# xingyizhou/CenterNet

Measured on AMD Instinct MI355X. Metric: images/sec whole-node, 512x512 ctdet, higher is better.
Workload: dtype f32s; 1 GPU; ctdet resdcn_18 512x512, batch 32 per GPU (BASELINE configs[1]), network + fused sigmoid/peak-NMS/top-K decode, K=100; global_batch=32, parallelism=image-sharded x1

## Files before the change

centernet_amd/csrc/cn_conv.hip:

```cpp
#include "cn_internal.h"
#include "cn_tuning.h"
#include <type_traits>

#ifndef CN_IGEMM_F32S_SETS
#define CN_IGEMM_F32S_SETS 1
#endif

namespace {

constexpr int NT = 256;
constexpr int BK = 32;
constexpr int LDT = BK + 4;

enum { A_DENSE = 0, A_STEM = 1, A_DCN = 2, A_DCN_PAD = 3 };
constexpr int STEM_KMAX = 512;

struct IgemmArgs {
    const void *x;
    const void *w;
    const float *bias;
    const float *scale;
    const float *shift;
    const void *residual;
    void *y;
// ... 850 lines not shown
extern "C" size_t cn_packed_conv_weight_elems(int Cout, int Cin, int KH, int KW, int dtype)
{
    const size_t n = packed_elems(Cout, Cin, KH, KW, dtype == CN_DTYPE_F16 ? 64 : 32);
    return (dtype == CN_DTYPE_F32S && ((KH == 3 && KW == 3) || (KH == 1 && KW == 1)) && Cin != 3) ? 2 * n : n;
}

template <typename T>
static int pack_conv_weight_t(const float *w_oihw, void *w_packed, int Cout, int Cin, int KH,
                              int KW, int bke, hipStream_t st)
{
    const int taps = KH * KW;
    const int cout_pad = round_up(Cout, 32);
    if (Cin == 3) {
        const int kpad = round_up(taps * 3, bke);
        const size_t total = (size_t)cout_pad * kpad;
        hipLaunchKernelGGL(pack_stem_weight_kernel<T>, dim3((unsigned)cn_cdiv((int)total, 256)),
                           dim3(256), 0, st, w_oihw, (T *)w_packed, Cout, taps, cout_pad, kpad);
    } else {
        const int cin_pad = round_up(Cin, bke);
        const size_t total = (size_t)taps * cout_pad * cin_pad;
        int blocks = (int)((total + 255) / 256);
        if (blocks > 4096) blocks = 4096;
        hipLaunchKernelGGL(pack_weight_kernel<T>, dim3(blocks), dim3(256), 0, st, w_oihw,
                           (T *)w_packed, Cout, Cin, taps, cout_pad, cin_pad);
    }
    CN_CHECK_LAUNCH();
    return CN_OK;
}

extern "C" int cn_pack_conv_weight(const float *w_oihw, void *w_packed, int Cout, int Cin, int KH,
                                   int KW, int dtype, void *stream)
{
    if (!w_oihw || !w_packed) return CN_ERR_NULL;
    if (Cout <= 0 || Cin <= 0 || KH <= 0 || KW <= 0) return CN_ERR_SHAPE;
    if (dtype == CN_DTYPE_F16)
        return pack_conv_weight_t<_Float16>(w_oihw, w_packed, Cout, Cin, KH, KW, 64, (hipStream_t)stream);
    if (dtype == CN_DTYPE_F32S && Cin != 3) {
        const int taps = KH * KW, cout_pad = round_up(Cout, 32), cin_pad = round_up(Cin, 32);
        const size_t total = (size_t)taps * cout_pad * cin_pad;
        int blocks = (int)((total + 255) / 256);
        if (blocks > 4096) blocks = 4096;
        hipLaunchKernelGGL(pack_weight_f32s_kernel, dim3(blocks), dim3(256), 0, (hipStream_t)stream,
                           w_oihw, (_Float16 *)w_packed, Cout, Cin, taps, cout_pad, cin_pad);
        CN_CHECK_LAUNCH();
        if ((KH == 3 && KW == 3) || (KH == 1 && KW == 1)) {
            hipLaunchKernelGGL(pack_weight_f32s_frag_kernel, dim3(blocks), dim3(256), 0,
                               (hipStream_t)stream, w_oihw, (_Float16 *)w_packed + 2 * total, Cout, Cin,
                               taps, cout_pad / 32, cin_pad / 32);
            CN_CHECK_LAUNCH();
        }
        return CN_OK;
    }
    if (dtype != CN_DTYPE_F32 && dtype != CN_DTYPE_F32S) return CN_ERR_UNSUPPORTED;
    return pack_conv_weight_t<float>(w_oihw, w_packed, Cout, Cin, KH, KW, 32, (hipStream_t)stream);
}

extern "C" int cn_pack_conv_weight_f32(const float *w_oihw, float *w_packed, int Cout, int Cin,
                                       int KH, int KW, void *stream)
{
    return cn_pack_conv_weight(w_oihw, w_packed, Cout, Cin, KH, KW, CN_DTYPE_F32, stream);
}

static int conv_fill_args(const cn_conv_desc *d, IgemmArgs *a)
{
    if (d->B <= 0 || d->H <= 0 || d->W <= 0 || d->Cin <= 0 || d->Cout <= 0 || d->KH <= 0 ||
        d->KW <= 0 || d->stride <= 0 || d->dil <= 0 || d->Ho <= 0 || d->Wo <= 0)
        return CN_ERR_SHAPE;
    const int ho = (d->H + 2 * d->pad_h - (d->dil * (d->KH - 1) + 1)) / d->stride + 1;
    const int wo = (d->W + 2 * d->pad_w - (d->dil * (d->KW - 1) + 1)) / d->stride + 1;
    if (d->oy_mul == 1 && d->ox_mul == 1 && (ho != d->Ho || wo != d->Wo)) return CN_ERR_SHAPE;
    if ((long)d->B * d->H * d->W * (long)(d->in_layout == CN_LAYOUT_NHWC ? d->in_pitch : d->Cin) >=
        (1L << 31))
        return CN_ERR_UNSUPPORTED;
    if ((long)d->B * d->OH * d->OW * (long)(d->out_layout == CN_LAYOUT_NHWC ? d->out_pitch : d->Cout) >=
        (1L << 31))
        return CN_ERR_UNSUPPORTED;
    a->B = d->B; a->H = d->H; a->W = d->W; a->Cin = d->Cin;
    a->Ho = d->Ho; a->Wo = d->Wo; a->Cout = d->Cout;
    a->KH = d->KH; a->KW = d->KW; a->stride = d->stride;
    a->pad_h = d->pad_h; a->pad_w = d->pad_w; a->dil = d->dil;
    a->in_pitch = d->in_pitch; a->out_pitch = d->out_pitch;
    a->OH = d->OH; a->OW = d->OW;
    a->oy_mul = d->oy_mul; a->oy_add = d->oy_add; a->ox_mul = d->ox_mul; a->ox_add = d->ox_add;
    a->relu = d->relu;
    a->M = d->B * d->Ho * d->Wo;
    a->cout_pad = round_up(d->Cout, 32);
    const int f16 = (d->dtype == CN_DTYPE_F16);
    const int f32s = (d->dtype == CN_DTYPE_F32S);
    if (d->dtype != CN_DTYPE_F32 && !f16 && !f32s) return CN_ERR_UNSUPPORTED;
    if (f32s && d->in_layout == CN_LAYOUT_NHWC && !(d->flags & CN_CONV_X_PLAIN) && (d->in_pitch & 31))
        return CN_ERR_UNSUPPORTED;
    if (f32s && d->out_layout == CN_LAYOUT_NHWC && !(d->flags & CN_CONV_Y_PLAIN) && (d->out_pitch & 31))
        return CN_ERR_UNSUPPORTED;
    const int bke = f16 ? 64 : 32, epv = f16 ? 8 : 4;
    if (is_stem(d->Cin, d->in_layout)) {
        a->cin_pad = round_up(d->KH * d->KW * 3, bke);
        if (a->cin_pad > STEM_KMAX) return CN_ERR_UNSUPPORTED;
        a->nchunk = a->cin_pad / bke;
        a->KT = a->nchunk;
    } else {
        if (d->in_layout != CN_LAYOUT_NHWC) return CN_ERR_UNSUPPORTED;
        if ((d->Cin % epv) || (d->in_pitch % epv) || d->in_pitch < d->Cin) return CN_ERR_UNSUPPORTED;
        a->cin_pad = round_up(d->Cin, bke);
        a->nchunk = a->cin_pad / bke;
        a->KT = d->KH * d->KW * a->nchunk;
    }
    return CN_OK;
}

static void dense_tile_class(const cn_conv_desc *d, const IgemmArgs &a, int *cls, bool *bm64)
{
    const int waste128 = cn_cdiv(d->Cout, 128) * 128 - d->Cout;
    const int waste64 = cn_cdiv(d->Cout, 64) * 64 - d->Cout;
    const bool narrow = !cn_knobs.narrow && (waste128 - waste64 >= 64);
    *cls = (d->Cout > 64 && !narrow) ? 2 : (d->Cout > 32 ? 1 : 0);
    const long wgs128 = (long)cn_cdiv(a.M, 128) * cn_cdiv(d->Cout, 128) * (a.zparity ? 4 : 1);
    *bm64 = (*cls == 2) && (cn_knobs.bm ? (cn_knobs.bm == 64) : (wgs128 < 1024 && wgs128 != 512));
}

static int dense_ksplit(const cn_conv_desc *d, const IgemmArgs &a)
{
    if (cn_knobs.nosplit || d->out_layout != CN_LAYOUT_NHWC || is_stem(d->Cin, d->in_layout) ||
        a.zparity)
        return 1;
    int cls;
    bool bm64;
    dense_tile_class(d, a, &cls, &bm64);
    const int bm = bm64 ? 64 : 128, bn = cls == 2 ? 128 : (cls == 1 ? 64 : 32);
    return plan_ksplit(a.M, d->Cout, a.KT, bm, bn);
}

static bool is_3x3s1(const cn_conv_desc *d)
{
    return d->KH == 3 && d->KW == 3 && d->stride == 1 && d->pad_h == 1 && d->pad_w == 1 && d->dil == 1 &&
           d->oy_mul == 1 && d->ox_mul == 1 && d->oy_add == 0 && d->ox_add == 0 && d->OH == d->Ho &&
           d->OW == d->Wo;
}

extern "C" int cn_conv2d_res_pitch_supported(const cn_conv_desc *d)
{
    IgemmArgs a = {};
    if (!d || conv_fill_args(d, &a) != CN_OK) return 0;
    if (cn_knobs.nohalo || !is_3x3s1(d) || is_stem(d->Cin, d->in_layout) || d->out_layout != CN_LAYOUT_NHWC) return 0;
    if (d->dtype == CN_DTYPE_F32 && d->Cin == 16 && d->Cout <= 32) return 0;
    if (d->dtype == CN_DTYPE_F32S && (d->flags & CN_CONV_X_PLAIN) && (d->flags & CN_CONV_Y_PLAIN) && d->Cin == 16 &&
        d->Cout <= 32)
        return 0;
    a.in_plain = (d->flags & CN_CONV_X_PLAIN) ? 1 : 0;
    a.out_plain = (d->flags & CN_CONV_Y_PLAIN) ? 1 : 0;
    a.res_plain = (d->flags & CN_CONV_R_PLAIN) ? 1 : 0;
    return dense_ksplit(d, a) > 1 ? 0 : 1;
}

extern "C" size_t cn_conv2d_workspace_bytes(const cn_conv_desc *d)
{
    IgemmArgs a = {};
    if (!d || conv_fill_args(d, &a) != CN_OK) return 0;
    const int s = dense_ksplit(d, a);
    return s > 1 ? (size_t)s * a.M * a.cout_pad * sizeof(float) : 0;
}

extern "C" int cn_conv2d(const cn_conv_desc *d, const void *x, const void *w_packed,
                         const float *scale, const float *shift, const void *residual, void *y,
                         void *workspace, size_t workspace_bytes, void *stream)
{
    if (!d || !x || !w_packed || !y) return CN_ERR_NULL;
    if (!cn_aligned16(x) || !cn_aligned16(w_packed)) return CN_ERR_ALIGN;
    IgemmArgs a = {};
    int rc = conv_fill_args(d, &a);
    if (rc != CN_OK) return rc;
    a.x = x; a.w = w_packed; a.bias = nullptr; a.scale = scale; a.shift = shift;
    a.residual = residual; a.y = y; a.om = nullptr;
    set_ctl(a, &d->ctl);
    if (d->dtype == CN_DTYPE_F32S) {
        if (d->in_layout == CN_LAYOUT_NHWC && !(d->flags & CN_CONV_X_PLAIN) && !aligned128(x)) return CN_ERR_ALIGN;
        if (d->out_layout == CN_LAYOUT_NHWC && !(d->flags & CN_CONV_Y_PLAIN) && !aligned128(y)) return CN_ERR_ALIGN;
        if (residual && !(d->flags & CN_CONV_R_PLAIN) && !aligned128(residual)) return CN_ERR_ALIGN;
    }
    const bool f16 = (d->dtype == CN_DTYPE_F16);
    const size_t valign = f16 ? 8 : 16;
    a.vec_out = (d->out_layout == CN_LAYOUT_NHWC && (d->out_pitch & 3) == 0 &&
                 (((uintptr_t)y) % valign) == 0 &&
                 (!residual || (((uintptr_t)residual) % valign) == 0)) ? 1 : 0;
    hipStream_t st = (hipStream_t)stream;
    const bool stem = is_stem(d->Cin, d->in_layout);
    const bool f32s = (d->dtype == CN_DTYPE_F32S);
    int cls;
    bool bm64;
    dense_tile_class(d, a, &cls, &bm64);
    a.ksplit = 1;
    a.in_plain = (d->flags & CN_CONV_X_PLAIN) ? 1 : 0;
    a.out_plain = (d->flags & CN_CONV_Y_PLAIN) ? 1 : 0;
    a.res_plain = (d->flags & CN_CONV_R_PLAIN) ? 1 : 0;
    const int want = dense_ksplit(d, a);
    if (want > 1 && workspace && cn_aligned16(workspace) &&
        workspace_bytes >= (size_t)want * a.M * a.cout_pad * sizeof(float)) {
        a.ksplit = want;
        a.partial = (float *)workspace;
    }
    if (f32s && stem) return CN_ERR_UNSUPPORTED;
    if (d->out_layout == CN_LAYOUT_NCHW) {
        if (residual || stem) return CN_ERR_UNSUPPORTED;
        if (f32s) {
            if (cls == 2) return launch_igemm_s<128, 128, 2, 2, A_DENSE, true>(a, st);
            if (cls == 1) return launch_igemm_s<128, 64, 2, 2, A_DENSE, true>(a, st);
            return launch_igemm_s<128, 32, 4, 1, A_DENSE, true>(a, st);
        }
        if (f16) {
            if (cls == 2) return launch_igemm_h<128, 128, 2, 2, A_DENSE, true>(a, st);
            if (cls == 1) return launch_igemm_h<128, 64, 2, 2, A_DENSE, true>(a, st);
            return launch_igemm_h<128, 32, 4, 1, A_DENSE, true>(a, st);
        }
        if (cls == 2) return launch_igemm<128, 128, 2, 2, A_DENSE, true>(a, st);
        if (cls == 1) return launch_igemm<128, 64, 2, 2, A_DENSE, true>(a, st);
        return launch_igemm<128, 32, 4, 1, A_DENSE, true>(a, st);
    }
    if (stem) {
        if (f16) {
            if (d->Cout > 64) return launch_igemm_h<128, 128, 2, 2, A_STEM, false>(a, st);
            if (d->Cout > 32) return launch_igemm_h<128, 64, 2, 2, A_STEM, false>(a, st);
            return launch_igemm_h<128, 32, 4, 1, A_STEM, false>(a, st);
        }
        if (d->flags & CN_CONV_STEM_MAXPOOL) {
            if (!(d->flags & CN_CONV_STEM_F32S) || residual || d->pad_h != d->pad_w || d->dil != 1)
                return CN_ERR_UNSUPPORTED;
            return cn_stem_pool_f32s((const float *)x, (const float *)w_packed, scale, shift,
                                     (float *)y, d->B, d->H, d->W, d->Ho, d->Wo, d->Cout, d->KH,
                                     d->KW, d->stride, d->pad_h, d->relu, d->out_pitch, a.cin_pad,
                                     (d->flags & CN_CONV_STEM_Y_F32S) ? 1 : 0, &d->ctl, st);
        }
        if (!cn_knobs.nostem && d->pad_h == d->pad_w && d->dil == 1 && d->oy_mul == 1 &&
            d->ox_mul == 1 && d->OH == d->Ho && d->OW == d->Wo) {
            rc = cn_stem_conv_f32((const float *)x, (const float *)w_packed, scale, shift,
                                  (float *)y, d->B, d->H, d->W, d->Ho, d->Wo, d->Cout, d->KH,
                                  d->KW, d->stride, d->pad_h, d->relu, d->out_pitch, a.cin_pad,
                                  cn_knobs.stem_persist | ((d->flags & CN_CONV_STEM_F32S) ? 2 : 0), &d->ctl, st);
            if (rc != CN_ERR_UNSUPPORTED) return rc;
        }
        if (d->Cout > 64) return launch_igemm<128, 128, 2, 2, A_STEM, false>(a, st);
        if (d->Cout > 32) return launch_igemm<128, 64, 2, 2, A_STEM, false>(a, st);
        return launch_igemm<128, 32, 4, 1, A_STEM, false>(a, st);
    }
    if (!cn_knobs.nohalo && !f16 && !f32s && !residual && a.ksplit == 1 && d->Cin == 16 && d->Cout <= 32 &&
        d->KH == 3 && d->KW == 3 && d->pad_h == 1 && d->pad_w == 1 && d->dil == 1 &&
        d->oy_mul == 1 && d->ox_mul == 1 && d->oy_add == 0 && d->ox_add == 0 && d->OH == d->Ho &&
        d->OW == d->Wo && d->in_layout == CN_LAYOUT_NHWC) {
        rc = cn_conv3x3_c16((const float *)x, (const float *)w_packed, scale, shift, (float *)y, d->B,
                            d->H, d->W, d->Ho, d->Wo, d->Cin, d->Cout, d->stride, d->in_pitch,
                            d->out_pitch, d->relu, st);
        if (rc != CN_ERR_UNSUPPORTED) return rc;
    }
    if (!cn_knobs.nohalo && f32s && (d->flags & CN_CONV_X_PLAIN) && (d->flags & CN_CONV_Y_PLAIN) && !residual &&
        a.ksplit == 1 && d->Cin == 16 && d->Cout <= 32 && d->KH == 3 && d->KW == 3 && d->pad_h == 1 &&
        d->pad_w == 1 && d->dil == 1 && d->oy_mul == 1 && d->ox_mul == 1 && d->oy_add == 0 &&
        d->ox_add == 0 && d->OH == d->Ho && d->OW == d->Wo && d->in_layout == CN_LAYOUT_NHWC) {
        rc = cn_conv3x3_c16s((const float *)x, w_packed, scale, shift, (float *)y, d->B, d->H, d->W,
                             d->Ho, d->Wo, d->Cin, d->Cout, d->stride, d->in_pitch, d->out_pitch,
                             d->relu, &d->ctl, st);
        if (rc != CN_ERR_UNSUPPORTED) return rc;
    }
    if (f32s && (d->flags & CN_CONV_X_PLAIN) && (d->flags & CN_CONV_Y_PLAIN) && !residual && is_3x3s1(d) &&
        d->in_layout == CN_LAYOUT_NHWC && d->out_layout == CN_LAYOUT_NHWC && a.vec_out &&
        cn_offconv_takes(d->B, d->H, d->W, d->Cin, d->Cout, d->in_pitch, d->out_pitch, a.ksplit)) {
        rc = cn_offconv_f32s((const float *)x, w_packed, scale, shift, (float *)y, d->B, d->H, d->W, d->Cin, d->Cout,
                             d->out_pitch, d->relu, &d->ctl, a.ksplit, a.partial, st);
        if (rc != CN_OK || a.ksplit == 1) return rc;
        const size_t tot = (size_t)a.M * (a.cout_pad >> 2);
        hipLaunchKernelGGL(splitk_reduce_kernel<cn_f32s>, dim3((unsigned)((tot + 255) / 256 < 8192 ? (tot + 255) / 256 : 8192)),
                           dim3(256), 0, st, a);
        CN_CHECK_LAUNCH();
        return CN_OK;
    }
    const int res_pitch = d->res_pitch > 0 ? d->res_pitch : d->out_pitch;
    const bool to_halo = !cn_knobs.nohalo && a.ksplit == 1 && is_3x3s1(d);
    if (residual && res_pitch != d->out_pitch && !to_halo) return CN_ERR_UNSUPPORTED;
    if (to_halo)
        return cn_conv3x3s1(x, w_packed, scale, shift, residual, y, d->B, d->H, d->W, d->Cin,
                            d->Cout, d->in_pitch, d->out_pitch, res_pitch, d->relu, a.vec_out, cls, d->dtype, d->flags,
                            &d->ctl, st);
    if (!cn_knobs.nohalo && f32s && !(d->flags & (CN_CONV_X_PLAIN | CN_CONV_R_PLAIN)) && !residual && scale &&
        a.vec_out && d->KH == 3 && d->KW == 3 && d->stride == 2 && d->pad_h == 1 && d->pad_w == 1 && d->dil == 1 &&
        d->oy_mul == 1 && d->ox_mul == 1 && d->oy_add == 0 && d->ox_add == 0 && d->OH == d->Ho && d->OW == d->Wo &&
        d->in_layout == CN_LAYOUT_NHWC && d->out_layout == CN_LAYOUT_NHWC &&
        cn_conv3x3s2p_takes(d->B, d->H, d->W, d->Cin, d->Cout, d->in_pitch, d->out_pitch))
        return cn_conv3x3s2_persist(x, w_packed, scale, shift, y, d->B, d->H, d->W, d->Cin, d->Cout, d->in_pitch,
                                    d->out_pitch, d->relu, (d->flags & CN_CONV_Y_PLAIN) ? 1 : 0, &d->ctl, st);
    if (f32s && !(d->flags & (CN_CONV_X_PLAIN | CN_CONV_R_PLAIN)) && !residual && scale && a.vec_out && d->KH == 1 &&
        d->KW == 1 && d->pad_h == 0 && d->pad_w == 0 && d->dil == 1 && d->oy_mul == 1 && d->ox_mul == 1 &&
        d->oy_add == 0 && d->ox_add == 0 && d->OH == d->Ho && d->OW == d->Wo && d->in_layout == CN_LAYOUT_NHWC &&
        d->out_layout == CN_LAYOUT_NHWC && d->Ho == (d->H - 1) / d->stride + 1 && d->Wo == (d->W - 1) / d->stride + 1 &&
        cn_proj1x1_takes(d->B, d->H, d->W, d->Cin, d->Cout, d->stride, d->in_pitch, d->out_pitch))
        return cn_proj1x1_f32s(x, w_packed, scale, shift, y, d->B, d->H, d->W, d->Cin, d->Cout, d->stride, d->in_pitch,
                               d->out_pitch, d->relu, (d->flags & CN_CONV_Y_PLAIN) ? 1 : 0, &d->ctl, st);
    if (f32s) {
        if (cls == 2)
            rc = bm64 ? launch_igemm_s<64, 128, 2, 2, A_DENSE, false>(a, st)
                      : launch_igemm_s<128, 128, 2, 2, A_DENSE, false>(a, st);
        else if (cls == 1)
            rc = launch_igemm_s<128, 64, 2, 2, A_DENSE, false>(a, st);
        else
            rc = launch_igemm_s<128, 32, 4, 1, A_DENSE, false>(a, st);
    } else if (f16) {
        if (cls == 2)
            rc = bm64 ? launch_igemm_h<64, 128, 2, 2, A_DENSE, false>(a, st)
                      : launch_igemm_h<128, 128, 2, 2, A_DENSE, false>(a, st);
        else if (cls == 1)
            rc = launch_igemm_h<128, 64, 2, 2, A_DENSE, false>(a, st);
        else
            rc = launch_igemm_h<128, 32, 4, 1, A_DENSE, false>(a, st);
    } else {
        if (cls == 2)
            rc = bm64 ? launch_igemm<64, 128, 2, 2, A_DENSE, false>(a, st)
                      : launch_igemm<128, 128, 2, 2, A_DENSE, false>(a, st);
        else if (cls == 1)
            rc = launch_igemm<128, 64, 2, 2, A_DENSE, false>(a, st);
        else
            rc = launch_igemm<128, 32, 4, 1, A_DENSE, false>(a, st);
    }
    if (rc != CN_OK || a.ksplit == 1) return rc;
    const size_t total = (size_t)a.M * (a.cout_pad >> 2);
    int blocks = (int)((total + 255) / 256);
    if (blocks > 8192) blocks = 8192;
    if (f32s)
        hipLaunchKernelGGL(splitk_reduce_kernel<cn_f32s>, dim3(blocks), dim3(256), 0, st, a);
    else if (f16)
        hipLaunchKernelGGL(splitk_reduce_kernel<_Float16>, dim3(blocks), dim3(256), 0, st, a);
    else
        hipLaunchKernelGGL(splitk_reduce_kernel<float>, dim3(blocks), dim3(256), 0, st, a);
    CN_CHECK_LAUNCH();
    return CN_OK;
// ... 338 lines not shown
```

centernet_amd/csrc/cn_conv3x3p.hip:

```cpp
#include "cn_internal.h"
#include "cn_tuning.h"
#include <type_traits>

__device__ __attribute__((aligned(128))) unsigned char cn_p3_zero_line[128];

namespace {

typedef __attribute__((address_space(3))) void p3_lds_void;
typedef __attribute__((address_space(1))) const void p3_gl_void;
typedef _Float16 p3_f16x8 __attribute__((ext_vector_type(8)));
typedef _Float16 p3_f16x4 __attribute__((ext_vector_type(4)));
typedef uint32_t p3_u32x2 __attribute__((ext_vector_type(2)));

constexpr int P_TH = 8, P_TW = 16;
constexpr int P_HW = P_TW + 2;
constexpr int P_HR = (P_TH + 2) * P_HW;
constexpr int P_HP = (P_HR + 7) / 8;
constexpr int P_HBYTES = P_HP * 1024;
constexpr int P_WSLOT = 64 * 128;
constexpr int P_NSLOT = 4;
constexpr int P_WOFF = 2 * P_HBYTES;
constexpr int P_SSOFF = P_WOFF + P_NSLOT * P_WSLOT;
constexpr int P_LDS = P_SSOFF + 6 * 256;
constexpr int P_STG_ROW = 144;
constexpr int P_STG = 32 * P_STG_ROW;
static_assert(4 * P_STG <= P_HBYTES, "the epilogue strips alias one halo buffer");
static_assert(P_LDS <= 81920, "two workgroups per CU");

struct P3Args {
    const char *x;
    const char *w;
    const float *scale, *shift;
    const char *residual;
    char *y;
    int H, W;
    int Hi, Wi;
    int in_pitchB, out_pitchB, res_pitchB;
    int res_bytes;
    int cin_padB;
    int cout_pad;
    int ngroups;
    int nchunk, nblk;
    int tiles_x, tiles_y;
    int items;
    int npar;
    int relu, out_plain, res_plain;
    float res_mul;
    uint32_t *range;
    int stagger;
    int knobs;
    int dbg;
    unsigned long long *prof;
};

__device__ __forceinline__ void p3_barrier()
{
    asm volatile("" ::: "memory");
    __builtin_amdgcn_s_barrier();
    asm volatile("" ::: "memory");
}

constexpr int P_MAXH = 8;
#ifndef P3_SPLIT
#define P3_SPLIT 4
#endif

static_assert(P3_SPLIT >= 4, "the front part of a block must reference all six fragments (see the fence in front of the barrier)");
struct P3Heads {
    const char *wf[P_MAXH];
    const float *bias[P_MAXH];
    const float *oscale[P_MAXH];
    float *y[P_MAXH];
    int cout[P_MAXH];
};

__device__ __forceinline__ void p3_lds_fence() { asm volatile("s_waitcnt lgkmcnt(0)" ::: "memory"); }

struct P3Item { int b, ty0, tx0, nb, par; };
__device__ __forceinline__ P3Item p3_decode(const P3Args &a, int item)
{
    P3Item it;
    it.nb = item % a.nblk;
    int t = item / a.nblk;
    it.par = t % a.npar;
    t /= a.npar;
    const int tx = t % a.tiles_x;
    t /= a.tiles_x;
    const int ty = t % a.tiles_y;
    it.b = t / a.tiles_y;
    it.ty0 = ty * P_TH;
    it.tx0 = tx * P_TW;
    return it;
}

__device__ constexpr int p3_s2_oy(int i) { return i == 0 || i == 1 || i == 6 ? 0 : 1; }
__device__ constexpr int p3_s2_ox(int i) { return i == 0 || i == 2 || i == 4 ? 0 : 1; }
__device__ constexpr int p3_s2_buf(int i) { return (i >= 4 && i <= 5) || i == 8 ? 1 : 0; }
__device__ constexpr int p3_s2_tap(int i)
{
    return i == 0 ? 0 : i == 1 ? 2 : i == 2 ? 6 : i == 3 ? 8 : i == 4 ? 3 : i == 5 ? 5 : i == 6 ? 1 : i == 7 ? 7 : 4;
}

#ifndef P3_HALO2
#define P3_HALO2 1
#endif

constexpr int p3_halo_loaders(int ntap, bool s2) { return (P3_HALO2 && (s2 || ntap == 4)) ? 2 : 1; }
constexpr int p3_threads(int ntap, bool s2) { return 320 + 64 * p3_halo_loaders(ntap, s2); }

template <int RES, bool OUT_PLAIN, bool DBG = false, bool HEADS = false, int NTAP = 9, bool S2 = false, bool PIPE = false>
__global__ __launch_bounds__(p3_threads(NTAP, S2), 4) void conv3x3p_kernel(const P3Args a, const P3Heads hd)
{
    static_assert(!PIPE || !DBG, "pipelined fragment schedule: not in the instrumented instantiation");
    static_assert(!S2 || (NTAP == 9 && RES == 0 && !DBG && !HEADS), "stride 2: nine taps, no residual");
    constexpr int RES_AT = 0;
    static_assert(!HEADS || (RES == 0 && !DBG), "fused heads: no residual, no probes");
    static_assert(NTAP == 9 || (NTAP == 4 && RES == 0 && !DBG && !HEADS), "4 taps: the transposed convolution's parity form");
    constexpr bool DECONV = (NTAP == 4);
    extern __shared__ __attribute__((aligned(128))) char smem[];
    const int tid = threadIdx.x, lane = tid & 63, wave = tid >> 6;

    const int nx = gridDim.x >> 3;
    const int xcd = blockIdx.x & 7, jx = blockIdx.x >> 3;
    const int per = (a.items + 7) >> 3;
    const int lo = xcd * per, hi = min(lo + per, a.items);
    const int first = lo + jx;
    const int nit = first < hi ? (hi - first + nx - 1) / nx : 0;
    if (nit == 0) return;
    const int S = nit * a.nchunk;

    unsigned long long pf_rt0 = 0;
    if (DBG) pf_rt0 = __builtin_amdgcn_s_memrealtime();
    if (a.stagger && blockIdx.x >= 256) {
        const unsigned long long t0 = __builtin_readcyclecounter();
        while (__builtin_readcyclecounter() - t0 < (unsigned long long)a.stagger * 256u) __builtin_amdgcn_s_sleep(32);
    }

    if (wave >= 4) {
        const int prow = lane >> 3, ps = lane & 7;
        unsigned long long pf_wait = 0, pf_bar = 0, pf_t0 = 0;
        auto now = [&]() { return DBG ? (unsigned long long)__builtin_readcyclecounter() : 0ull; };
        if (DBG) pf_t0 = now();
        __builtin_amdgcn_s_setprio(3);
#define P3_IC(v) std::integral_constant<int, (v)>{}
        if (wave == 4) {
            unsigned wofs[8];
            auto set_wofs = [&](int nb) {
#pragma unroll
                for (int p = 0; p < 8; ++p) {
                    const int n = 8 * p + prow;
                    const int row = min(nb * 64 + n, a.cout_pad - 1);
                    wofs[p] = (unsigned)(row * a.cin_padB + ((ps ^ ((n >> 1) & 7)) << 4));
                }
            };
            set_wofs(first % a.nblk);
            const size_t tapB = (size_t)a.cout_pad * a.cin_padB;
            int wk = 0, wc = 0, wt = 0, wg = 0;
            size_t wpar = DECONV ? (size_t)((first / a.nblk) % a.npar) * NTAP * tapB : 0;
            auto issue_W = [&]() {
                if (wk >= nit) return;
                const char *base = a.w + wpar + (size_t)(S2 ? p3_s2_tap(wt) : wt) * tapB + (size_t)wc * 128;
                char *dst = smem + P_WOFF + (wg & (P_NSLOT - 1)) * P_WSLOT;
                if (!DBG || !(a.dbg & 4)) {
#pragma unroll
                    for (int p = 0; p < 8; ++p)
                        __builtin_amdgcn_global_load_lds((p3_gl_void *)(base + wofs[p]), (p3_lds_void *)(dst + p * 1024), 16, 0, 0);
                }
                ++wg;
                if (++wt == NTAP) {
                    wt = 0;
                    if (++wc == a.nchunk) {
                        wc = 0;
                        ++wk;
                        if (wk < nit && a.nblk > 1) set_wofs((first + wk * nx) % a.nblk);
                        if (DECONV && wk < nit) wpar = (size_t)(((first + wk * nx) / a.nblk) % a.npar) * NTAP * tapB;
                    }
                }
            };
            issue_W();
            issue_W();
            issue_W();
            for (int s = 0;; ++s) {
                const bool last = (s >= S - 1);
#pragma unroll
                for (int t = 0; t < NTAP; ++t) {
                    const unsigned long long c0 = now();
                    if (last) asm volatile("s_waitcnt vmcnt(0)" ::: "memory");
                    else asm volatile("s_waitcnt vmcnt(16)" ::: "memory");
                    const unsigned long long c1 = now();
                    p3_barrier();
                    if (DBG) { pf_wait += c1 - c0; pf_bar += now() - c1; }
                    if (s == S) break;
                    issue_W();
                }
                if (s == S) break;
            }
        } else {
            auto halo_loader = [&](auto HW) {
            constexpr int NHL = p3_halo_loaders(NTAP, S2), NPW = (P_HP + NHL - 1) / NHL;
            constexpr int hw = decltype(HW)::value;
            int poff[NPW];
            int pyx[NPW];
#pragma unroll
            for (int j = 0; j < NPW; ++j) {
                const int k = j * NHL + hw;
                const int r = 8 * k + prow;
                const int hy = r / P_HW, hx = r - hy * P_HW;
                const int col = ps ^ ((hx >> 1) & 7);
                poff[j] = (S2 ? 2 : 1) * ((hy - 1) * a.Wi + (hx - 1)) * a.in_pitchB + col * 16;
                pyx[j] = (r < P_HR) ? (hy | (hx << 8)) : -1;
            }
            const char *zero = reinterpret_cast<const char *>(cn_p3_zero_line) + ps * 16;
            int hk = 0, hc = 0, hj = 0;
            int hp = S2 ? 1 : 0, hq = S2 ? 1 : 0;
            P3Item hit = p3_decode(a, first);
            const char *hbase = nullptr;
            auto set_hbase = [&]() {
                if constexpr (S2) {
                    hp = (hj == 0 || hj == 2) ? 1 : 0;
                    hq = (hj == 0 || hj == 1) ? 1 : 0;
                    hbase = a.x + ((size_t)(hit.b * a.Hi + 2 * hit.ty0 + hp) * a.Wi + 2 * hit.tx0 + hq) * a.in_pitchB +
                            (size_t)hc * 128;
                } else {
                    hbase = a.x + ((size_t)(hit.b * a.Hi + hit.ty0) * a.Wi + hit.tx0) * a.in_pitchB + (size_t)hc * 128;
                }
            };
            set_hbase();
            auto issue_H = [&](auto K0, auto K1, int buf) {
                constexpr int k0 = decltype(K0)::value, k1 = decltype(K1)::value;
                char *dst = smem + buf * P_HBYTES;
                if (DBG && (a.dbg & 8)) return;
#pragma unroll
                for (int j = k0 / NHL; j < (k1 + NHL - 1) / NHL; ++j) {
                    const int k = j * NHL + hw;
                    if (NHL == 2 && (k < k0 || k >= k1)) continue;
                    const int hy = pyx[j] & 255, hx = pyx[j] >> 8;
                    const int iy = S2 ? 2 * (hit.ty0 - 1 + hy) + hp : hit.ty0 - 1 + hy;
                    const int ix = S2 ? 2 * (hit.tx0 - 1 + hx) + hq : hit.tx0 - 1 + hx;
                    const bool ok = pyx[j] >= 0 && (unsigned)iy < (unsigned)a.Hi && (unsigned)ix < (unsigned)a.Wi;
                    const char *src = ok ? hbase + poff[j] : zero;
                    __builtin_amdgcn_global_load_lds((p3_gl_void *)src, (p3_lds_void *)(dst + k * 1024), 16, 0, 0);
                }
            };
            auto advance_H = [&]() {
                if (S2 && ++hj < 4) {
                    set_hbase();
                    return;
                }
                hj = 0;
                if (++hc == a.nchunk) {
                    hc = 0;
                    ++hk;
                    if (hk < nit) hit = p3_decode(a, first + hk * nx);
                }
                if (hk < nit) set_hbase();
            };
            issue_H(P3_IC(0), P3_IC(P_HP), 0);
            advance_H();
            if constexpr (S2) {
                const int ST = 4 * S;
                bool done = false;
                auto run_stage = [&](auto N, int s) {
                    constexpr int n = decltype(N)::value;
                    const bool last = (s >= ST - 1);
                    const int nbuf = (s + 1) & 1;
#pragma unroll
                    for (int t = 0; t < n; ++t) {
                        if (t == 0) asm volatile("s_waitcnt vmcnt(0)" ::: "memory");
                        p3_barrier();
                        if (s == ST) { done = true; return; }
                        if (!last) {
                            if constexpr (n == 4) {
                                if (t == 1) issue_H(P3_IC(0), P3_IC(12), nbuf);
                                if (t == 2) issue_H(P3_IC(12), P3_IC(P_HP), nbuf);
                            } else if constexpr (n == 2) {
                                if (t == 0) issue_H(P3_IC(0), P3_IC(P_HP), nbuf);
                            } else {
                                issue_H(P3_IC(0), P3_IC(P_HP), nbuf);
                            }
                        }
                    }
                };
                for (int s = 0;; ++s) {
                    const int sj = s & 3;
                    if (sj == 0) run_stage(P3_IC(4), s);
                    else if (sj == 3) run_stage(P3_IC(1), s);
                    else run_stage(P3_IC(2), s);
                    if (done) break;
                    if (s < ST - 1) advance_H();
                }
            } else
            for (int s = 0;; ++s) {
                const bool last = (s >= S - 1);
                const int nbuf = (s + 1) & 1;
#pragma unroll
                for (int t = 0; t < NTAP; ++t) {
                    const unsigned long long c0 = now();
                    if (t == 0) asm volatile("s_waitcnt vmcnt(0)" ::: "memory");
                    const unsigned long long c1 = now();
                    p3_barrier();
                    if (DBG) { pf_wait += c1 - c0; pf_bar += now() - c1; }
                    if (s == S) break;
                    if (!last) {
                        if constexpr (DECONV) {
                            if (t == 1) issue_H(P3_IC(0), P3_IC(12), nbuf);
                            if (t == 2) issue_H(P3_IC(12), P3_IC(P_HP), nbuf);
                        } else {
                            if (t == 1) issue_H(P3_IC(0), P3_IC(4), nbuf);
                            if (t == 2) issue_H(P3_IC(4), P3_IC(8), nbuf);
                            if (t == 3) issue_H(P3_IC(8), P3_IC(12), nbuf);
                            if (t == 4) issue_H(P3_IC(12), P3_IC(16), nbuf);
                            if (t == 5) issue_H(P3_IC(16), P3_IC(20), nbuf);
                            if (t == 6) issue_H(P3_IC(20), P3_IC(P_HP), nbuf);
                        }
                    }
                }
                if (s == S) break;
                if (!last) advance_H();
            }
            };
            if (p3_halo_loaders(NTAP, S2) == 1 || wave == 5) halo_loader(P3_IC(0));
            else halo_loader(P3_IC(1));
        }
#undef P3_IC
        if (DBG && a.prof && lane == 0) {
            unsigned long long *o = a.prof + ((size_t)blockIdx.x * 6 + wave) * 8;
            o[0] = now() - pf_t0; o[1] = pf_wait; o[2] = pf_bar; o[3] = (unsigned long long)S;
            o[4] = pf_rt0; o[5] = __builtin_amdgcn_s_memrealtime();
        }
        return;
    }


    if constexpr (HEADS) {
        int arow, aswz, b0;
        auto lane_consts = [&]() {
            int ln = lane;
            asm volatile("" : "+v"(ln));
            const int l31 = ln & 31, lh = ln >> 5, px = ln & 15;
            arow = ((2 * wave + (l31 >> 4)) * P_HW + px) * 128;
            aswz = 0;
#pragma unroll
            for (int kx = 0; kx < 3; ++kx) aswz |= (((lh ^ (((px + kx) >> 1) & 7)) & 7) << 4) << (8 * kx);
            b0 = l31 * 128 + (((lh ^ ((l31 >> 1) & 7)) & 7) << 4);
        };
        lane_consts();
        cn_f32x16 acc[2];
        auto zero_acc = [&]() {
#pragma unroll
            for (int j = 0; j < 2; ++j)
#pragma unroll
                for (int r = 0; r < 16; ++r) acc[j][r] = 0.f;
        };
        zero_acc();
        float rng_out = 0.f;
        auto lds128 = [&](int off) { return *reinterpret_cast<const p3_f16x8 *>(smem + off); };
        auto step = [&](auto T, int hb, int wb) {
            constexpr int t = decltype(T)::value;
            constexpr int ky = t / 3, kx = t % 3;
            constexpr int tapoff = (ky * P_HW + kx) * 128;
            constexpr int blk1 = 32 * 128;
            p3_f16x8 xf[4], wf[4][2];
            int ax = arow + ((aswz >> (8 * kx)) & 0xff), bx = b0;
            asm volatile("" : "+v"(ax), "+v"(bx));
#pragma unroll
            for (int kh = 0; kh < 2; ++kh) {
#pragma unroll
                for (int j = 0; j < 2; ++j) wf[kh][j] = lds128(wb + j * blk1 + (bx ^ (kh << 5)));
                xf[2 + kh] = lds128(hb + tapoff + (ax ^ ((kh << 5) | 64)));
                xf[kh] = lds128(hb + tapoff + (ax ^ (kh << 5)));
#pragma unroll
                for (int j = 0; j < 2; ++j) wf[2 + kh][j] = lds128(wb + j * blk1 + (bx ^ ((kh << 5) | 64)));
            }
            __builtin_amdgcn_sched_barrier(0);
            if (!(a.knobs & 1)) __builtin_amdgcn_s_setprio(1);
#pragma unroll
            for (int kh = 0; kh < 2; ++kh) {
#pragma unroll
                for (int j = 0; j < 2; ++j)
                    acc[j] = __builtin_amdgcn_mfma_f32_32x32x16_f16(wf[kh][j], xf[2 + kh], acc[j], 0, 0, 0);
#pragma unroll
                for (int j = 0; j < 2; ++j)
                    acc[j] = __builtin_amdgcn_mfma_f32_32x32x16_f16(wf[2 + kh][j], xf[kh], acc[j], 0, 0, 0);
#pragma unroll
                for (int j = 0; j < 2; ++j)
                    acc[j] = __builtin_amdgcn_mfma_f32_32x32x16_f16(wf[kh][j], xf[kh], acc[j], 0, 0, 0);
            }
            if (!(a.knobs & 1)) __builtin_amdgcn_s_setprio(0);
        };
        const float relu_floor = a.relu ? 0.f : -__builtin_inff();
        const int HWp = a.H * a.W;
        auto load_w2 = [&](p3_f16x8 (&dst)[2][2], const char *wbase, int jb, int j, int ln) {
#pragma unroll
            for (int s2 = 0; s2 < 2; ++s2)
#pragma unroll
                for (int part = 0; part < 2; ++part)
                    dst[s2][part] = *reinterpret_cast<const p3_f16x8 *>(
                        wbase + ((((jb * 2 + j) * 2 + s2) * 2 + part) * 64 + ln) * 16);
        };
        p3_f16x8 wfa[2][2], wfb[2][2];
        auto epilogue = [&](const P3Item &it) {
            int ln = lane;
            asm volatile("" : "+v"(ln));
            const int l31 = ln & 31, lh = ln >> 5;
            const int head = it.nb;
            const int cout2 = hd.cout[head];
            const char *w2 = hd.wf[head];
            float *y2 = hd.y[head];
            const int nblk2 = (cout2 + 31) >> 5;
            p3_f16x8 shi[2][2], slo[2][2];
#pragma unroll
            for (int j = 0; j < 2; ++j) {
// ... 371 lines not shown
        const int grp = 2 * it.nb + wn;
#pragma unroll
        for (int i = 0; i < 2; ++i)
#pragma unroll
            for (int k = 0; k < 4; ++k) {
                bool ok;
                const int pix = row_pixel(it, i, k, rrow, ok);
                const bool take = ok && grp < a.ngroups;
                const unsigned off = take ? (unsigned)pix * (unsigned)a.res_pitchB + (unsigned)(grp * 128 + rcol * 16) : 0u;
                resv[i][k] = __builtin_bit_cast(cn_f32x4, __builtin_amdgcn_raw_buffer_load_b128(res_rsrc, off, 0, 0));
            }
    };

    const float relu_floor = a.relu ? 0.f : -__builtin_inff();
    auto epilogue = [&](const P3Item &it, int sb) {
        const int grp = 2 * it.nb + wn;
        if (grp >= a.ngroups) return;
        const int stg = sb + wave * P_STG;
        const int ln = opaque_lane();
        const int rrow = ln >> 3, rcol = ln & 7, l31 = ln & 31, lh = ln >> 5;
        const int rowb = stg + l31 * P_STG_ROW + 8 * lh;
#pragma unroll
        for (int i = 0; i < 2; ++i) {
            if constexpr (RES != 0) {
#pragma unroll
                for (int k = 0; k < 4; ++k)
                    *reinterpret_cast<cn_f32x4 *>(smem + stg + (8 * k + rrow) * P_STG_ROW + rcol * 16) = resv[i][k];
                asm volatile("" ::: "memory");
            }
            cn_f32x4 rr[4];
            if constexpr (RES != 0) {
#pragma unroll
                for (int g = 0; g < 4; ++g) {
                    if constexpr (RES == 2)
                        rr[g] = *reinterpret_cast<const cn_f32x4 *>(smem + rowb + 8 * lh + 32 * g);
                    else
                        rr[g] = cn_join4(*reinterpret_cast<const cn_f16x4v *>(smem + rowb + 16 * g),
                                         *reinterpret_cast<const cn_f16x4v *>(smem + rowb + 64 + 16 * g));
                }
                asm volatile("" ::: "memory");
            }
#pragma unroll
            for (int g = 0; g < 4; ++g) {
                const cn_f32x4 sc = *reinterpret_cast<const cn_f32x4 *>(smem + P_SSOFF + wave * 256 + (8 * g + 4 * lh) * 4);
                const cn_f32x4 sh = *reinterpret_cast<const cn_f32x4 *>(smem + P_SSOFF + wave * 256 + 128 + (8 * g + 4 * lh) * 4);
                cn_f32x4 v;
#pragma unroll
                for (int e = 0; e < 4; ++e) v[e] = acc[i][4 * g + e] * sc[e] + sh[e];
                if constexpr (RES != 0) {
#pragma unroll
                    for (int e = 0; e < 4; ++e) v[e] = fmaf(rr[g][e], a.res_mul, v[e]);
                }
#pragma unroll
                for (int e = 0; e < 4; ++e) v[e] = fmaxf(v[e], relu_floor);
                if constexpr (OUT_PLAIN) {
                    *reinterpret_cast<cn_f32x4 *>(smem + rowb + 8 * lh + 32 * g) = v;
                } else {
                    cn_rng_upd4(rng_out, v);
                    cn_f16x4v h4, l4;
                    cn_split4(v, h4, l4);
                    *reinterpret_cast<cn_f16x4v *>(smem + rowb + 16 * g) = h4;
                    *reinterpret_cast<cn_f16x4v *>(smem + rowb + 64 + 16 * g) = l4;
                }
            }
            asm volatile("" ::: "memory");
#pragma unroll
            for (int k = 0; k < 4; ++k) {
                bool ok;
                const int pix = row_pixel(it, i, k, rrow, ok);
                const cn_f32x4 v = *reinterpret_cast<const cn_f32x4 *>(smem + stg + (8 * k + rrow) * P_STG_ROW + rcol * 16);
                if (ok && !(DBG && (a.dbg & 32)))
                    *reinterpret_cast<cn_f32x4 *>(a.y + ((unsigned)pix * (unsigned)a.out_pitchB + (unsigned)(grp * 128 + rcol * 16))) = v;
            }
            asm volatile("" ::: "memory");
        }
    };

    P3Item cur = p3_decode(a, first), prev = cur;
    par_y = cur.par >> 1; par_x = cur.par & 1;
    int k = 0, c = 0, g = 0;
    unsigned long long pf_bar = 0, pf_epi = 0, pf_t0 = 0;
    auto now = [&]() { return DBG ? (unsigned long long)__builtin_readcyclecounter() : 0ull; };
    if (DBG) pf_t0 = now();
    auto bar = [&]() {
        const unsigned long long c0 = now();
        p3_barrier();
        if (DBG) pf_bar += now() - c0;
    };
#define P3_IC(v) std::integral_constant<int, (v)>{}
    if constexpr (PIPE) {
        struct Frag { p3_f16x8 wh, wl, xh[2], xl[2]; };
        Frag F0, F1;
        auto load_half = [&](auto T, auto KH, int hb, int wb, Frag &F) {
            constexpr int t = decltype(T)::value, kh = decltype(KH)::value;
            const int ky = S2 ? p3_s2_oy(t) : (DECONV ? t / 2 + par_y : t / 3);
            const int kx = S2 ? p3_s2_ox(t) : (DECONV ? t % 2 + par_x : t % 3);
            const int tapoff = (ky * P_HW + kx) * 128;
            int ax = arow + ((aswz >> (8 * kx)) & 0xff) + (DECONV ? tapoff : 0), bx = b0;
            asm volatile("" : "+v"(ax), "+v"(bx));
            const int tapimm = DECONV ? 0 : tapoff;
            constexpr int blk1 = 2 * P_HW * 128;
            F.wh = lds128(wb + (bx ^ (kh << 5)));
#pragma unroll
            for (int i = 0; i < 2; ++i) F.xl[i] = lds128(hb + tapimm + i * blk1 + (ax ^ ((kh << 5) | 64)));
#pragma unroll
            for (int i = 0; i < 2; ++i) F.xh[i] = lds128(hb + tapimm + i * blk1 + (ax ^ (kh << 5)));
            F.wl = lds128(wb + (bx ^ ((kh << 5) | 64)));
        };
        auto mfma_front = [&](const Frag &F) {
#pragma unroll
            for (int i = 0; i < 2; ++i) acc[i] = __builtin_amdgcn_mfma_f32_32x32x16_f16(F.wh, F.xl[i], acc[i], 0, 0, 0);
            if constexpr (P3_SPLIT >= 4) {
#pragma unroll
                for (int i = 0; i < 2; ++i) acc[i] = __builtin_amdgcn_mfma_f32_32x32x16_f16(F.wl, F.xh[i], acc[i], 0, 0, 0);
            }
            if constexpr (P3_SPLIT >= 6) {
#pragma unroll
                for (int i = 0; i < 2; ++i) acc[i] = __builtin_amdgcn_mfma_f32_32x32x16_f16(F.wh, F.xh[i], acc[i], 0, 0, 0);
            }
        };
        auto mfma_back = [&](const Frag &F) {
            if constexpr (P3_SPLIT < 4) {
#pragma unroll
                for (int i = 0; i < 2; ++i) acc[i] = __builtin_amdgcn_mfma_f32_32x32x16_f16(F.wl, F.xh[i], acc[i], 0, 0, 0);
            }
            if constexpr (P3_SPLIT < 6) {
#pragma unroll
                for (int i = 0; i < 2; ++i) acc[i] = __builtin_amdgcn_mfma_f32_32x32x16_f16(F.wh, F.xh[i], acc[i], 0, 0, 0);
            }
        };
        auto keep = [&](const Frag &F) {
            asm volatile("" :: "v"(F.wh), "v"(F.wl), "v"(F.xh[0]), "v"(F.xh[1]), "v"(F.xl[0]), "v"(F.xl[1]));
        };
        bar();
        int s = 0;
        for (k = 0; k < nit; ++k) {
            cur = p3_decode(a, first + k * nx);
            par_y = cur.par >> 1; par_x = cur.par & 1;
            float ssv;
            {
                const int grp = 2 * cur.nb + wn;
                const int ln = opaque_lane();
                const unsigned o = (unsigned)(32 * grp + (ln & 31)) * 4u;
                float sv = 1.f, hv = 0.f;
                if (grp < a.ngroups) {
                    sv = *reinterpret_cast<const float *>(reinterpret_cast<const char *>(a.scale) + o);
                    if (a.shift) hv = *reinterpret_cast<const float *>(reinterpret_cast<const char *>(a.shift) + o);
                }
                ssv = (ln >> 5) ? hv : sv;
            }
            __builtin_amdgcn_sched_barrier(0);
            load_half(P3_IC(0), P3_IC(0), S2 ? 0 : (s & 1) * P_HBYTES, P_WOFF + (g & 3) * P_WSLOT, F0);
            __builtin_amdgcn_sched_barrier(0);
            for (c = 0; c < a.nchunk; ++c, ++s) {
                const int hb0 = (s & 1) * P_HBYTES, hb1 = ((s + 1) & 1) * P_HBYTES;
                auto HB = [&](int i) { return S2 ? p3_s2_buf(i) * P_HBYTES : hb0; };
                auto WB = [&](int i) { return P_WOFF + ((g + i) & 3) * P_WSLOT; };
                const bool more = (c + 1 < a.nchunk);
                auto pstep = [&](auto T) {
                    constexpr int t = decltype(T)::value;
                    __builtin_amdgcn_sched_barrier(0);
                    __builtin_amdgcn_s_setprio(1);
                    mfma_front(F0);
                    __builtin_amdgcn_sched_barrier(0);
                    load_half(T, P3_IC(1), HB(t), WB(t), F1);
                    __builtin_amdgcn_sched_barrier(0);
                    keep(F0);
                    mfma_back(F0);
                    __builtin_amdgcn_sched_barrier(0);
                    mfma_front(F1);
                    __builtin_amdgcn_sched_barrier(0);
                    __builtin_amdgcn_s_setprio(0);
                    p3_lds_fence();
                    p3_barrier();
                    if constexpr (t + 1 < NTAP) {
                        load_half(P3_IC(t + 1), P3_IC(0), HB(t + 1), WB(t + 1), F0);
                    } else {
                        if (more) load_half(P3_IC(0), P3_IC(0), S2 ? 0 : hb1, WB(NTAP), F0);
                    }
                    __builtin_amdgcn_sched_barrier(0);
                    keep(F1);
                    mfma_back(F1);
                    __builtin_amdgcn_sched_barrier(0);
                };
                pstep(P3_IC(0));
                pstep(P3_IC(1));
                pstep(P3_IC(2));
                if (c == 0) *reinterpret_cast<float *>(smem + P_SSOFF + wave * 256 + lane * 4) = ssv;
                pstep(P3_IC(3));
                if constexpr (!DECONV) {
                    pstep(P3_IC(4));
                    pstep(P3_IC(5));
                    pstep(P3_IC(6));
                    pstep(P3_IC(7));
                    pstep(P3_IC(8));
                }
                g += NTAP;
            }
            if constexpr (RES != 0) {
                __builtin_amdgcn_sched_barrier(0);
                load_residual(cur);
                __builtin_amdgcn_sched_barrier(0);
            }
            epilogue(cur, S2 ? P_HBYTES : ((s - 1) & 1) * P_HBYTES);
            zero_acc();
            lane_consts();
        }
    } else
    for (int s = 0;; ++s) {
        bar();
        if (s > 0 && c == 0) {
            const unsigned long long c0 = now();
            if (!(DBG && (a.dbg & 16))) epilogue(prev, S2 ? P_HBYTES : ((s - 1) & 1) * P_HBYTES);
            zero_acc();
            lane_consts();
            if (DBG) pf_epi += now() - c0;
        }
        if (s == S) break;
        const int hb0 = (s & 1) * P_HBYTES;
        auto HB = [&](int i) { return S2 ? p3_s2_buf(i) * P_HBYTES : hb0; };
        float ssv = 0.f;
        if (c == 0) {
            const int grp = 2 * cur.nb + wn;
            const int ln = opaque_lane();
            const unsigned o = (unsigned)(32 * grp + (ln & 31)) * 4u;
            float sv = 1.f, hv = 0.f;
            if (grp < a.ngroups) {
                sv = *reinterpret_cast<const float *>(reinterpret_cast<const char *>(a.scale) + o);
                if (a.shift) hv = *reinterpret_cast<const float *>(reinterpret_cast<const char *>(a.shift) + o);
            }
            ssv = (ln >> 5) ? hv : sv;
        }
        step(P3_IC(0), HB(0), P_WOFF + ((g + 0) & 3) * P_WSLOT);
        bar(); step(P3_IC(1), HB(1), P_WOFF + ((g + 1) & 3) * P_WSLOT);
        bar(); step(P3_IC(2), HB(2), P_WOFF + ((g + 2) & 3) * P_WSLOT);
        if (c == 0) *reinterpret_cast<float *>(smem + P_SSOFF + wave * 256 + lane * 4) = ssv;
        bar(); step(P3_IC(3), HB(3), P_WOFF + ((g + 3) & 3) * P_WSLOT);
        if constexpr (!DECONV) {
        bar(); step(P3_IC(4), HB(4), P_WOFF + ((g + 4) & 3) * P_WSLOT);
        bar(); step(P3_IC(5), HB(5), P_WOFF + ((g + 5) & 3) * P_WSLOT);
        auto maybe_residual = [&](int at) {
            if constexpr (RES != 0) {
                if (at == RES_AT && c == a.nchunk - 1) {
                    __builtin_amdgcn_sched_barrier(0);
                    load_residual(cur);
                    __builtin_amdgcn_sched_barrier(0);
                }
            }
        };
        maybe_residual(3);
        bar(); step(P3_IC(6), HB(6), P_WOFF + ((g + 6) & 3) * P_WSLOT);
        maybe_residual(2);
        bar(); step(P3_IC(7), HB(7), P_WOFF + ((g + 7) & 3) * P_WSLOT);
        maybe_residual(1);
        bar(); step(P3_IC(8), HB(8), P_WOFF + ((g + 8) & 3) * P_WSLOT);
        maybe_residual(0);
        }
        g += NTAP;
        if (++c == a.nchunk) {
            c = 0;
            prev = cur;
            ++k;
            if (k < nit) cur = p3_decode(a, first + k * nx);
            par_y = cur.par >> 1; par_x = cur.par & 1;
        }
    }
    if (DBG && a.prof && lane == 0) {
        unsigned long long *o = a.prof + ((size_t)blockIdx.x * 6 + wave) * 8;
        o[0] = now() - pf_t0; o[1] = pf_epi; o[2] = pf_bar; o[3] = (unsigned long long)S;
        o[4] = pf_rt0; o[5] = __builtin_amdgcn_s_memrealtime();
        unsigned xcc;
        asm volatile("s_getreg_b32 %0, hwreg(HW_REG_XCC_ID)" : "=s"(xcc));
        unsigned hwid;
        asm volatile("s_getreg_b32 %0, hwreg(HW_REG_HW_ID)" : "=s"(hwid));
        o[6] = xcc; o[7] = hwid;
    }
#undef P3_IC
    if constexpr (!OUT_PLAIN) {
        if (a.range) cn_rng_commit(a.range, 0, rng_out);
    }
}

}

bool cn_conv3x3p_takes(int B, int H, int W, int Cin, int Cout, int in_pitch, int out_pitch, int res_pitch,
                       bool in_plain, bool has_res)
{
    if (!cn_knobs.c3p || in_plain) return false;
    if ((in_pitch & 31) || (out_pitch & 31) || (has_res && (res_pitch & 31))) return false;
    if (Cout % 32) return false;
    const long items = (long)B * cn_cdiv(H, P_TH) * cn_cdiv(W, P_TW) * cn_cdiv(Cout, 64);
    if (cn_knobs.c3p < 2 && items < 256) return false;
    if ((long)B * H * W * (long)max(in_pitch, max(out_pitch, res_pitch)) * 4 >= (1L << 31)) return false;
    (void)Cin;
    return true;
}

bool cn_deconv4x4s2p_takes(int B, int H, int W, int Cin, int Cout, int in_pitch, int out_pitch, bool in_plain)
{
    if (!cn_knobs.c3p || !(cn_knobs.c3p_deconv) || in_plain) return false;
    if ((in_pitch & 31) || (out_pitch & 31) || (Cout % 32)) return false;
    const long items = 4L * B * cn_cdiv(H, P_TH) * cn_cdiv(W, P_TW) * cn_cdiv(Cout, 64);
    if (cn_knobs.c3p < 2 && items < 256) return false;
    if (4L * B * H * W * (long)max(in_pitch, out_pitch) * 4 >= (1L << 31)) return false;
    (void)Cin;
    return true;
}

int cn_deconv4x4s2_persist(const void *x, const void *w_packed, const float *scale, const float *shift, void *y,
                           int B, int H, int W, int Cin, int Cout, int in_pitch, int out_pitch, int relu,
                           int out_plain, const cn_f32s_ctl *ctl, hipStream_t st)
{
    P3Args a = {};
    a.x = (const char *)x; a.w = (const char *)w_packed; a.scale = scale; a.shift = shift;
    a.y = (char *)y;
    a.H = H; a.W = W;
    a.Hi = H; a.Wi = W;
    a.in_pitchB = in_pitch * 4; a.out_pitchB = out_pitch * 4;
    const int cin_pad = (Cin + 31) / 32 * 32;
    a.cin_padB = cin_pad * 4;
    a.cout_pad = (Cout + 31) / 32 * 32;
    a.ngroups = a.cout_pad / 32;
    a.nchunk = cin_pad / 32;
    a.nblk = cn_cdiv(Cout, 64);
    a.npar = 4;
    a.tiles_x = cn_cdiv(W, P_TW);
    a.tiles_y = cn_cdiv(H, P_TH);
    a.items = B * a.tiles_y * a.tiles_x * a.npar * a.nblk;
    a.relu = relu; a.out_plain = out_plain;
    a.res_mul = 1.f;
    a.range = ctl ? ctl->range : nullptr;
    a.stagger = cn_knobs.c3p_stagger;
    a.knobs = cn_knobs.c3p_knobs;
    int per_xcd = cn_cdiv(a.items, 8);
    if (per_xcd > 64) per_xcd = 64;
    const dim3 grid(8 * per_xcd), block(p3_threads(4, false));
#define P3_LAUNCH4(OP, PIPE)                                                                                     \
    do {                                                                                                         \
        CN_SET_MAX_LDS_ONCE((conv3x3p_kernel<0, OP, false, false, 4, false, PIPE>), P_LDS);                       \
        hipLaunchKernelGGL((conv3x3p_kernel<0, OP, false, false, 4, false, PIPE>), grid, block, P_LDS, st, a, P3Heads{}); \
    } while (0)
    if (a.knobs & 2) {
        if (out_plain) P3_LAUNCH4(true, true); else P3_LAUNCH4(false, true);
    } else {
        if (out_plain) P3_LAUNCH4(true, false); else P3_LAUNCH4(false, false);
    }
#undef P3_LAUNCH4
    CN_CHECK_LAUNCH();
    return CN_OK;
}

bool cn_conv3x3s2p_takes(int B, int Hi, int Wi, int Cin, int Cout, int in_pitch, int out_pitch)
{
    if (!cn_knobs.c3p || !cn_knobs.c3p_s2) return false;
    if ((in_pitch & 31) || (out_pitch & 31) || (Cout % 32)) return false;
    const int Ho = (Hi - 1) / 2 + 1, Wo = (Wi - 1) / 2 + 1;
    const long items = (long)B * cn_cdiv(Ho, P_TH) * cn_cdiv(Wo, P_TW) * cn_cdiv(Cout, 64);
    if (cn_knobs.c3p < 2 && items < 256) return false;
    if ((long)B * Hi * Wi * (long)in_pitch * 4 >= (1L << 31) || (long)B * Ho * Wo * (long)out_pitch * 4 >= (1L << 31))
        return false;
    (void)Cin;
    return true;
}

int cn_conv3x3s2_persist(const void *x, const void *w_packed, const float *scale, const float *shift, void *y,
                         int B, int Hi, int Wi, int Cin, int Cout, int in_pitch, int out_pitch, int relu,
                         int out_plain, const cn_f32s_ctl *ctl, hipStream_t st)
{
    P3Args a = {};
    a.x = (const char *)x; a.w = (const char *)w_packed; a.scale = scale; a.shift = shift;
    a.y = (char *)y;
    a.H = (Hi - 1) / 2 + 1; a.W = (Wi - 1) / 2 + 1;
    a.Hi = Hi; a.Wi = Wi;
    a.in_pitchB = in_pitch * 4; a.out_pitchB = out_pitch * 4;
    const int cin_pad = (Cin + 31) / 32 * 32;
    a.cin_padB = cin_pad * 4;
    a.cout_pad = (Cout + 31) / 32 * 32;
    a.ngroups = a.cout_pad / 32;
    a.nchunk = cin_pad / 32;
    a.nblk = cn_cdiv(Cout, 64);
    a.npar = 1;
    a.tiles_x = cn_cdiv(a.W, P_TW);
    a.tiles_y = cn_cdiv(a.H, P_TH);
    a.items = B * a.tiles_y * a.tiles_x * a.nblk;
    a.relu = relu; a.out_plain = out_plain;
    a.res_mul = 1.f;
    a.range = ctl ? ctl->range : nullptr;
    a.stagger = cn_knobs.c3p_stagger;
    a.knobs = cn_knobs.c3p_knobs;
    int per_xcd = cn_cdiv(a.items, 8);
    if (per_xcd > 64) per_xcd = 64;
    const dim3 grid(8 * per_xcd), block(p3_threads(9, true));
#define P3_LAUNCHS2(OP, PIPE)                                                                                    \
    do {                                                                                                         \
        CN_SET_MAX_LDS_ONCE((conv3x3p_kernel<0, OP, false, false, 9, true, PIPE>), P_LDS);                        \
        hipLaunchKernelGGL((conv3x3p_kernel<0, OP, false, false, 9, true, PIPE>), grid, block, P_LDS, st, a, P3Heads{}); \
    } while (0)
    if (a.knobs & 2) {
        if (out_plain) P3_LAUNCHS2(true, true); else P3_LAUNCHS2(false, true);
    } else {
        if (out_plain) P3_LAUNCHS2(true, false); else P3_LAUNCHS2(false, false);
    }
#undef P3_LAUNCHS2
    CN_CHECK_LAUNCH();
    return CN_OK;
}

static int p3_probe_dbg = 0;
static unsigned long long *p3_probe_prof = nullptr;
extern "C" int cn_conv3x3p_occupancy(int res, int out_plain)
{
    int n = -1;
    hipError_t e;
#define P3_OCC(R, OP)                                                                             \
    do {                                                                                          \
        CN_SET_MAX_LDS_ONCE((conv3x3p_kernel<R, OP>), P_LDS);                                      \
        e = hipOccupancyMaxActiveBlocksPerMultiprocessor(&n, conv3x3p_kernel<R, OP>, 384, P_LDS);  \
    } while (0)
    if (out_plain) {
        if (res == 0) P3_OCC(0, true); else if (res == 1) P3_OCC(1, true); else P3_OCC(2, true);
    } else {
        if (res == 0) P3_OCC(0, false); else if (res == 1) P3_OCC(1, false); else P3_OCC(2, false);
    }
#undef P3_OCC
    return e == hipSuccess ? n : -(int)e;
}

extern "C" int cn_conv3x3p_probe(int dbg, void *prof)
{
    p3_probe_dbg = dbg;
    p3_probe_prof = (unsigned long long *)prof;
    return CN_OK;
}

int cn_conv3x3s1_persist(const void *x, const void *w_packed, const float *scale, const float *shift,
                         const void *residual, void *y, int B, int H, int W, int Cin, int Cout,
                         int in_pitch, int out_pitch, int res_pitch, int relu, int out_plain, int res_plain,
                         const cn_f32s_ctl *ctl, hipStream_t st)
{
    P3Args a = {};
    a.x = (const char *)x; a.w = (const char *)w_packed; a.scale = scale; a.shift = shift;
    a.residual = (const char *)residual; a.y = (char *)y;
    a.H = H; a.W = W;
    a.Hi = H; a.Wi = W;
    a.in_pitchB = in_pitch * 4; a.out_pitchB = out_pitch * 4; a.res_pitchB = res_pitch * 4;
    a.res_bytes = (int)((long)B * H * W * res_pitch * 4);
    const int cin_pad = (Cin + 31) / 32 * 32;
    a.cin_padB = cin_pad * 4;
    a.cout_pad = (Cout + 31) / 32 * 32;
    a.ngroups = a.cout_pad / 32;
    a.nchunk = cin_pad / 32;
    a.nblk = cn_cdiv(Cout, 64);
    a.npar = 1;
    a.tiles_x = cn_cdiv(W, P_TW);
    a.tiles_y = cn_cdiv(H, P_TH);
    a.items = B * a.tiles_y * a.tiles_x * a.nblk;
    a.relu = relu; a.out_plain = out_plain; a.res_plain = res_plain;
    a.res_mul = (ctl && ctl->res_mul != 0.f) ? ctl->res_mul : 1.f;
    a.range = ctl ? ctl->range : nullptr;
    a.stagger = cn_knobs.c3p_stagger;
    a.knobs = cn_knobs.c3p_knobs;
    int per_xcd = cn_cdiv(a.items, 8);
    if (per_xcd > 64) per_xcd = 64;
    const dim3 grid(8 * per_xcd), block(384);
#define P3_LAUNCH_(R, OP, PIPE)                                                                                  \
    do {                                                                                                         \
        CN_SET_MAX_LDS_ONCE((conv3x3p_kernel<R, OP, false, false, 9, false, PIPE>), P_LDS);                       \
        hipLaunchKernelGGL((conv3x3p_kernel<R, OP, false, false, 9, false, PIPE>), grid, block, P_LDS, st, a, P3Heads{}); \
    } while (0)
#define P3_LAUNCH(R, OP)                                                    \
    do {                                                                    \
        if (a.knobs & 2) P3_LAUNCH_(R, OP, true); else P3_LAUNCH_(R, OP, false); \
    } while (0)
    const int rmode = !residual ? 0 : (res_plain ? 2 : 1);
    if ((p3_probe_dbg || p3_probe_prof) && !out_plain && rmode < 2) {
        a.dbg = p3_probe_dbg;
        a.prof = p3_probe_prof;
        if (rmode == 0) {
            CN_SET_MAX_LDS_ONCE((conv3x3p_kernel<0, false, true>), P_LDS);
            hipLaunchKernelGGL((conv3x3p_kernel<0, false, true>), grid, block, P_LDS, st, a, P3Heads{});
        } else {
            CN_SET_MAX_LDS_ONCE((conv3x3p_kernel<1, false, true>), P_LDS);
            hipLaunchKernelGGL((conv3x3p_kernel<1, false, true>), grid, block, P_LDS, st, a, P3Heads{});
        }
        CN_CHECK_LAUNCH();
        return CN_OK;
    }
    if (out_plain) {
        if (rmode == 0) P3_LAUNCH(0, true); else if (rmode == 1) P3_LAUNCH(1, true); else P3_LAUNCH(2, true);
    } else {
        if (rmode == 0) P3_LAUNCH(0, false); else if (rmode == 1) P3_LAUNCH(1, false); else P3_LAUNCH(2, false);
    }
#undef P3_LAUNCH
#undef P3_LAUNCH_
    CN_CHECK_LAUNCH();
    return CN_OK;
}

bool cn_heads3x3p_takes(int B, int H, int W, int in_pitch, int head_conv, int n_heads, const cn_head_out *heads,
                        bool in_plain)
{
    if (!cn_knobs.c3p || !cn_knobs.c3p_heads || in_plain || head_conv != 64 || n_heads > P_MAXH) return false;
    if (in_pitch & 31) return false;
    for (int h = 0; h < n_heads; ++h)
        if (heads[h].cout > 96 || !heads[h].w_frag || !cn_aligned16(heads[h].w_frag)) return false;
    const long items = (long)B * cn_cdiv(H, P_TH) * cn_cdiv(W, P_TW) * n_heads;
    if (cn_knobs.c3p < 2 && items < 256) return false;
    if ((long)B * H * W * (long)in_pitch * 4 >= (1L << 31)) return false;
    for (int h = 0; h < n_heads; ++h)
        if ((long)B * heads[h].cout * H * W >= (1L << 31)) return false;
    return true;
}

int cn_heads3x3p(const void *x, int B, int H, int W, int Cin, int in_pitch, const void *w1_packed,
                 const float *scale1, const float *bias1, int n_heads, const cn_head_out *heads,
                 const cn_f32s_ctl *ctl, hipStream_t st)
{
    P3Args a = {};
    P3Heads hd = {};
    for (int h = 0; h < n_heads; ++h) {
        hd.wf[h] = (const char *)heads[h].w_frag; hd.bias[h] = heads[h].bias; hd.oscale[h] = heads[h].oscale;
        hd.y[h] = heads[h].y; hd.cout[h] = heads[h].cout;
    }
    a.x = (const char *)x; a.w = (const char *)w1_packed; a.scale = scale1; a.shift = bias1;
    a.H = H; a.W = W;
    a.Hi = H; a.Wi = W;
    a.in_pitchB = in_pitch * 4;
    const int cin_pad = (Cin + 31) / 32 * 32;
    a.cin_padB = cin_pad * 4;
    a.cout_pad = 64 * n_heads;
    a.ngroups = a.cout_pad / 32;
    a.nchunk = cin_pad / 32;
    a.nblk = n_heads;
    a.npar = 1;
    a.tiles_x = cn_cdiv(W, P_TW);
    a.tiles_y = cn_cdiv(H, P_TH);
    a.items = B * a.tiles_y * a.tiles_x * a.nblk;
    a.relu = 1;
    a.res_mul = 1.f;
    a.range = ctl ? ctl->range : nullptr;
    a.stagger = cn_knobs.c3p_stagger;
    a.knobs = cn_knobs.c3p_knobs;
    int per_xcd = cn_cdiv(a.items, 8);
    if (per_xcd > 64) per_xcd = 64;
    const dim3 grid(8 * per_xcd), block(384);
    a.knobs |= 2;
    CN_SET_MAX_LDS_ONCE((conv3x3p_kernel<0, false, false, true, 9, false, true>), P_LDS);
    hipLaunchKernelGGL((conv3x3p_kernel<0, false, false, true, 9, false, true>), grid, block, P_LDS, st, a, hd);
    CN_CHECK_LAUNCH();
    return CN_OK;
}

namespace {
__global__ void pack_head_w2_kernel(const float *__restrict__ w, char *__restrict__ out, int cout, int nblk2)
{
    const int t = blockIdx.x * blockDim.x + threadIdx.x;
    if (t >= nblk2 * 4 * 64) return;
    const int ln = t & 63, s2 = (t >> 6) & 1, j = (t >> 7) & 1, jb = t >> 8;
    const int l31 = ln & 31, lh = ln >> 5;
    const int row = jb * 32 + l31;
    _Float16 hi[8], lo[8];
#pragma unroll
    for (int q = 0; q < 8; ++q) {
        const int k = 32 * j + 16 * s2 + 8 * (q >> 2) + 4 * lh + (q & 3);
        const float v = row < cout ? w[(size_t)row * 64 + k] : 0.f;
        const float c = fminf(fmaxf(v, -65504.0f), 65504.0f);
        hi[q] = (_Float16)c;
        lo[q] = (_Float16)(c - (float)hi[q]);
    }
    char *o = out + ((size_t)((jb * 2 + j) * 2 + s2) * 2 * 64 + ln) * 16;
    *reinterpret_cast<p3_f16x8 *>(o) = *reinterpret_cast<const p3_f16x8 *>(hi);
    *reinterpret_cast<p3_f16x8 *>(o + 64 * 16) = *reinterpret_cast<const p3_f16x8 *>(lo);
}
}

extern "C" size_t cn_packed_head_w2_bytes(int cout)
{
    return cout > 0 ? (size_t)((cout + 31) / 32) * 8192 : 0;
}

extern "C" int cn_pack_head_w2_f32s(const float *w, void *out, int cout, void *stream)
{
    if (!w || !out) return CN_ERR_NULL;
    if (cout <= 0) return CN_ERR_SHAPE;
    if (!cn_aligned16(out)) return CN_ERR_ALIGN;
    const int nblk2 = (cout + 31) / 32;
    hipLaunchKernelGGL(pack_head_w2_kernel, dim3(nblk2), dim3(256), 0, (hipStream_t)stream, w, (char *)out, cout, nblk2);
    CN_CHECK_LAUNCH();
    return CN_OK;
}
```

centernet_amd/csrc/cn_internal.h:

```cpp
#pragma once
#include "cn_common.h"

int cn_stem_conv_f32(const float *x, const float *w_packed, const float *scale, const float *shift,
                     float *y, int B, int H, int W, int Ho, int Wo, int Cout, int KH, int KW,
                     int stride, int pad, int relu, int out_pitch, int KP, int persistent,
                     const cn_f32s_ctl *ctl, hipStream_t st);
int cn_stem_pool_rows(int B, int Ho, int Wo, int Cout, int KH, int KW, int stride, int KP);
int cn_stem_pool_f32s(const float *x, const float *w_packed, const float *scale, const float *shift,
                      float *y, int B, int H, int W, int Ho, int Wo, int Cout, int KH, int KW,
                      int stride, int pad, int relu, int out_pitch, int KP, int y_f32s, const cn_f32s_ctl *ctl,
                      hipStream_t st);

struct DcnWinCall {
    const float *x;
    const void *w;
    const float *bias, *om;
    int om_pitch;
    const float *scale, *shift;
    void *y;
    int out_pitch, out_plain;
    int B, Cin, H, W, Cout, mask_sigmoid, relu;
    float x_mul;
    uint32_t *range;
    int dbg;
    float *partial;
    size_t partial_bytes;
};
int cn_dcn_window_f32s(const DcnWinCall &c, int min_wgs, int *ksplit_out, hipStream_t st);
int cn_dcn_team_f32s(const DcnWinCall &c, int nmode, int *ksplit_out, hipStream_t st);
int cn_dcn_wide_f32s(const DcnWinCall &c, int nb, int *ksplit_out, hipStream_t st);

int cn_dcn_general_launch(const float *input, const float *weight, const float *bias,
                          const float *offset, const float *mask, float *output, int B, int Cin,
                          int H, int W, int Cout, int kh, int kw, int sh, int sw, int ph, int pw,
                          int dh, int dw, int dg, int mask_sigmoid, hipStream_t st);

bool cn_offconv_takes(int B, int H, int W, int Cin, int Cout, int in_pitch, int out_pitch, int ksplit);
int cn_offconv_f32s(const float *x, const void *w_packed, const float *scale, const float *shift, float *y,
                    int B, int H, int W, int Cin, int Cout, int out_pitch, int relu, const cn_f32s_ctl *ctl,
                    int ksplit, float *partial, hipStream_t st);

bool cn_proj1x1_takes(int B, int H, int W, int Cin, int Cout, int stride, int in_pitch, int out_pitch);
int cn_proj1x1_f32s(const void *x, const void *w_packed, const float *scale, const float *shift, void *y, int B, int H,
                    int W, int Cin, int Cout, int stride, int in_pitch, int out_pitch, int relu, int out_plain,
                    const cn_f32s_ctl *ctl, hipStream_t st);

int cn_conv3x3_c16(const float *x, const float *w_packed, const float *scale, const float *shift,
                   float *y, int B, int H, int W, int Ho, int Wo, int Cin, int Cout, int stride,
                   int in_pitch, int out_pitch, int relu, hipStream_t st);
int cn_conv3x3_c16s(const float *x, const void *w_packed, const float *scale, const float *shift,
                    float *y, int B, int H, int W, int Ho, int Wo, int Cin, int Cout, int stride,
                    int in_pitch, int out_pitch, int relu, const cn_f32s_ctl *ctl, hipStream_t st);

int cn_conv3x3s1(const void *x, const void *w_packed, const float *scale, const float *shift,
                 const void *residual, void *y, int B, int H, int W, int Cin, int Cout,
                 int in_pitch, int out_pitch, int res_pitch, int relu, int vec_out, int bn_class,
                 int dtype, int flags, const cn_f32s_ctl *ctl, hipStream_t st);
int cn_deconv4x4s2_halo(const void *x, const void *w_packed, const float *scale, const float *shift,
                        void *y, int B, int H, int W, int Cin, int Cout, int in_pitch, int out_pitch,
                        int relu, int vec_out, int dtype, int flags, const cn_f32s_ctl *ctl,
                        hipStream_t st);

bool cn_conv3x3p_takes(int B, int H, int W, int Cin, int Cout, int in_pitch, int out_pitch, int res_pitch,
                       bool in_plain, bool has_res);
int cn_conv3x3s1_persist(const void *x, const void *w_packed, const float *scale, const float *shift,
                         const void *residual, void *y, int B, int H, int W, int Cin, int Cout,
                         int in_pitch, int out_pitch, int res_pitch, int relu, int out_plain, int res_plain,
                         const cn_f32s_ctl *ctl, hipStream_t st);
bool cn_conv3x3s2p_takes(int B, int Hi, int Wi, int Cin, int Cout, int in_pitch, int out_pitch);
int cn_conv3x3s2_persist(const void *x, const void *w_packed, const float *scale, const float *shift, void *y,
                         int B, int Hi, int Wi, int Cin, int Cout, int in_pitch, int out_pitch, int relu,
                         int out_plain, const cn_f32s_ctl *ctl, hipStream_t st);
bool cn_deconv4x4s2p_takes(int B, int H, int W, int Cin, int Cout, int in_pitch, int out_pitch, bool in_plain);
int cn_deconv4x4s2_persist(const void *x, const void *w_packed, const float *scale, const float *shift, void *y,
                           int B, int H, int W, int Cin, int Cout, int in_pitch, int out_pitch, int relu,
                           int out_plain, const cn_f32s_ctl *ctl, hipStream_t st);
bool cn_heads3x3p_takes(int B, int H, int W, int in_pitch, int head_conv, int n_heads, const cn_head_out *heads,
                        bool in_plain);
int cn_heads3x3p(const void *x, int B, int H, int W, int Cin, int in_pitch, const void *w1_packed,
                 const float *scale1, const float *bias1, int n_heads, const cn_head_out *heads,
                 const cn_f32s_ctl *ctl, hipStream_t st);
```

centernet_amd/engine.py:

```python
import ctypes
import math
import os
import warnings

import torch

from . import native
from .native import (ConvDesc, F32sCtl, LAYOUT_NCHW, LAYOUT_NHWC, DTYPE_F16, DTYPE_F32, DTYPE_F32S,
                     CONV_X_PLAIN, CONV_Y_PLAIN, CONV_R_PLAIN, CONV_STEM_F32S,
                     CONV_STEM_MAXPOOL, CONV_STEM_Y_F32S)

TOP_LOG2 = 10
F16_MAX = 65504.0
LOW_WATER = 2.0 ** -3
LOW_STEP = 6
LOW_EVERY = 64
F16_MAX_BITS = 0x477FE000
LOW_WATER_BITS = 0x3E000000
W_TOP_LOG2 = 14


def exponent_for(absmax):
    if math.isinf(absmax) or math.isnan(absmax):
        raise native.NativeError("non-finite activations in the f32s calibration pass")
    if not absmax > 0.0:
        return 0
    return math.frexp(absmax)[1] - TOP_LOG2


def _out_size(n, k, s, p, d=1):
    return (n + 2 * p - (d * (k - 1) + 1)) // s + 1


class Act:
    __slots__ = ("t", "B", "H", "W", "C", "pitch", "c_off", "nchw", "fmt", "exp", "lid")

    def __init__(self, t, B, H, W, C, pitch=None, c_off=0, nchw=False, fmt="f32", exp=0, lid=None):
        self.t, self.B, self.H, self.W, self.C = t, B, H, W, C
        self.pitch = C if pitch is None else pitch
        self.c_off = c_off
        self.nchw = nchw
        self.fmt = fmt
        self.exp = exp
        self.lid = lid

    @property
    def applied_exp(self):
        return self.exp if self.fmt == "f32s" else 0

    def ptr(self):
        return ctypes.c_void_p(self.t.data_ptr() + self.t.element_size() * self.c_off)

    def to_float(self):
        t = self.t
        if self.nchw:
            return t.permute(0, 2, 3, 1).float()
        if self.fmt == "f32s":
            h = t.view(torch.float16).reshape(self.B, self.H, self.W, self.pitch // 32, 2, 32)
            t = (h[..., 0, :].float() + h[..., 1, :].float()).reshape(self.B, self.H, self.W,
                                                                      self.pitch)
            t = torch.ldexp(t, torch.tensor(self.exp))
        return t[..., self.c_off:self.c_off + self.C].float()


def prescale_rows(w):
    w = w.detach().float()
    m = w.abs().flatten(1).amax(dim=1)
    e = torch.frexp(m.clamp_min(1e-30))[1] - W_TOP_LOG2
    e = torch.where(m > 0, e, torch.zeros_like(e))
    shape = (-1,) + (1,) * (w.dim() - 1)
    return torch.ldexp(w, (-e).view(shape).expand_as(w)), torch.ldexp(torch.ones_like(m), e)


def _pow2(e):
    return math.ldexp(1.0, int(e))


def pack_cell_heads(firsts, lasts, device):
    lib = native.lib()
    w = torch.cat([c.weight.detach() for c in firsts], 0).to(device=device, dtype=torch.float32).contiguous()
    b1 = torch.cat([c.bias.detach() for c in firsts], 0).to(device=device, dtype=torch.float32).contiguous()
    N, ci = int(w.shape[0]), int(w.shape[1])
    hidden = int(firsts[0].weight.shape[0])
    w1 = torch.empty((9 * ci // 4, N, 4), device=device, dtype=torch.float32)
    native.check(lib.cn_pack_cell_heads_w1(native.ptr(w), native.ptr(w1), N, ci, native.stream_ptr()),
                 "cn_pack_cell_heads_w1")
    w2 = torch.stack([c.weight.detach().reshape(2, hidden) for c in lasts], 0)
    w2 = w2.to(device=device, dtype=torch.float32).contiguous()
    b2 = torch.stack([torch.zeros(2) if c.bias is None else c.bias.detach().cpu().float() for c in lasts], 0)
    b2 = b2.to(device=device, dtype=torch.float32).contiguous()
    return w1, b1, w2, b2


class DeferredHeads:
    __slots__ = ("names", "feat", "hidden", "w1", "b1", "w2", "b2")

    def __init__(self, names, feat, hidden, w1, b1, w2, b2):
        self.names, self.feat, self.hidden = tuple(names), feat, int(hidden)
        self.w1, self.b1, self.w2, self.b2 = w1, b1, w2, b2


def fold_bn(conv_bias, bn, cout, device):
    if bn is None:
        if conv_bias is None:
            return None, None
        return None, conv_bias.detach().to(device=device, dtype=torch.float32).contiguous()
    g = bn.weight.detach().float() if bn.weight is not None else torch.ones(cout)
    b = bn.bias.detach().float() if bn.bias is not None else torch.zeros(cout)
    mean = bn.running_mean.detach().float()
    var = bn.running_var.detach().float()
    scale = g / torch.sqrt(var + bn.eps)
    shift = b - mean * scale
    if conv_bias is not None:
        shift = shift + conv_bias.detach().float() * scale
    return (scale.to(device).contiguous(), shift.to(device).contiguous())


class PlanBuilder:

    RANGE_LAUNCHES = 256
    RANGE_WORDS = 2 * 64 * 16

    def __init__(self, device, B, H, W, dtype=torch.float32, wcache=None, split=None, exps=None,
                 calibrating=False, track=None, defer=()):
        assert dtype in (torch.float32, torch.float16)
        self.device = device
        self.defer = () if calibrating else tuple(defer)
        self.deferred = None
        if split is None:
            split = os.environ.get("CN_F32S", "1") != "0"
        self.split = bool(split) and dtype == torch.float32 and not calibrating
        self.calibrating = calibrating
        self.exps = dict(exps) if exps else {}
        self.wcache = wcache if wcache is not None else {}
        self.dtype = dtype
        self.cdtype = DTYPE_F16 if dtype == torch.float16 else DTYPE_F32
        self.B, self.H, self.W = B, H, W
        self.lib = native.lib()
        self.ops = []
        self.meta = []
        self.keep = []
        self.flops = 0
        self.input = None
        self.trace = []
        self.ws = None
        self.fuse_heads = os.environ.get("CN_FUSE_HEADS", "1") != "0" and not calibrating
        self.ws_bytes = 0
        self._nlid = 0
        self.groups = []
        self.range = None
        self.range_chunks = []
        self._plain_cache = {}
        self.range_slots = []
        self._pack_events = []
        if track is None:
            track = os.environ.get("CN_RANGE", "1") != "0"
        self.track = self.split and bool(track)

    def _lid(self, lid=None, tag=""):
        if lid is not None:
            return lid
        self._nlid += 1
        return "t%d%s" % (self._nlid, tag)

    def _exp(self, lid):
        return int(self.exps.get(lid, 0)) if self.split else 0

    def _ctl(self, lid, x_mul=1.0, res_mul=1.0):
        c = F32sCtl()
        c.x_mul, c.res_mul = float(x_mul), float(res_mul)
        c.range = None
        if self.track:
            slot = len(self.range_slots)
            ci, si = divmod(slot, self.RANGE_LAUNCHES)
            if ci == len(self.range_chunks):
                cur = torch.zeros((self.RANGE_LAUNCHES, self.RANGE_WORDS), device=self.device, dtype=torch.int32)
                stat = torch.zeros((2, self.RANGE_LAUNCHES, 2), device=self.device, dtype=torch.int32)
                stat[1].fill_(0x7f800000)
                self.range_chunks.append((cur, stat))
                if self.range is None:
                    self.range, self.range_stat = cur, stat
                    self.range_sum = torch.tensor([0, 0x7f800000], device=self.device, dtype=torch.int32)
                    self.range_sum_host = torch.tensor([0, 0x7f800000], dtype=torch.int32).pin_memory()
                    self.range_sum_event = torch.cuda.Event()
            self.range_slots.append(lid)
            c.range = self.range_chunks[ci][0].data_ptr() + 4 * self.RANGE_WORDS * si
        self.keep.append(c)
        return c

    def _new(self, B, H, W, C, pitch=None, fmt=None, lid=None):
        if fmt is None:
            fmt = "f16" if self.dtype == torch.float16 else "f32"
        pitch = C if pitch is None else pitch
        if fmt == "f32s":
            pitch = (pitch + 31) // 32 * 32
            t = torch.zeros((B, H, W, pitch), device=self.device, dtype=torch.float32)
        else:
            t = torch.empty((B, H, W, pitch), device=self.device, dtype=self.dtype)
        return Act(t, B, H, W, C, pitch, fmt=fmt, exp=self._exp(lid), lid=lid)

    def plain(self, x):
        if x is None or x.fmt != "f32s":
            return x
        assert x.c_off % 32 == 0
        key = (id(x.t), x.c_off, x.C)
        hit = self._plain_cache.get(key)
        if hit is not None and hit[0] is x.t:
            return hit[1]
        out = self._new(x.B, x.H, x.W, x.C, fmt="f32", lid=x.lid)
        out.exp = x.exp
        lib, npix = self.lib, x.B * x.H * x.W
        mul = _pow2(x.exp)

        def run():
            rc = lib.cn_f32s_to_f32_scaled(x.ptr(), out.ptr(), npix, x.C, x.pitch, out.pitch, mul,
                                           native.stream_ptr())
            if rc:
                native.check(rc, "cn_f32s_to_f32")
        self._emit_simple(run, "convert", out, 8 * npix * x.C)
        self._plain_cache[key] = (x.t, out)
        return out

    def packed(self, x):
        if x is None or x.fmt == "f32s":
            return x
        assert x.fmt == "f32" and not x.nchw
        out = self._new(x.B, x.H, x.W, x.C, fmt="f32s", lid=x.lid)
        out.exp = x.exp
        lib, npix = self.lib, x.B * x.H * x.W
        src = Act(x.t, x.B, x.H, x.W, x.C, x.pitch, x.c_off)
        ctl = self._ctl(x.lid)
        mul = _pow2(-x.exp)

        def run():
            rc = lib.cn_f32_to_f32s_scaled(src.ptr(), out.ptr(), npix, x.C, x.pitch, out.pitch, mul,
                                           ctl.range, native.stream_ptr())
            if rc:
                native.check(rc, "cn_f32_to_f32s")
        self._emit_simple(run, "convert", out, 8 * npix * x.C)
        return out

    def _wkey(self, kind, sources):
        return (kind, self.cdtype, str(self.device)) + tuple(
            (id(t), t._version, t.data_ptr(), tuple(t.shape)) for t in sources)

    def _wput(self, key, hit):
        ids = tuple(e[0] for e in key[3:])
        for k in [k for k in self.wcache if k[:3] == key[:3] and tuple(e[0] for e in k[3:]) == ids]:
            del self.wcache[k]
        self.wcache[key] = hit

    def _pack(self, w_oihw, sources=None, f32s=False, prescale=False):
        if sources is None:
            sources = [w_oihw]
        cacheable = all(isinstance(t, torch.nn.Parameter) for t in sources)
        kind = "conv_f32s" if f32s else ("conv_pre" if prescale else "conv")
        key = self._wkey(kind, sources) if cacheable else None
        hit = self.wcache.get(key) if cacheable else None
        if hit is None:
            w = w_oihw.detach().to(device=self.device, dtype=torch.float32).contiguous()
            factor = None
            if f32s or prescale:
                w, factor = prescale_rows(w)
                w = w.contiguous()
            cd = DTYPE_F32S if f32s else self.cdtype
            co, ci, kh, kw = w.shape
            n = self.lib.cn_packed_conv_weight_elems(co, ci, kh, kw, cd)
            wp = torch.empty(n, device=self.device, dtype=torch.float32 if f32s else self.dtype)
            native.check(self.lib.cn_pack_conv_weight(native.ptr(w), native.ptr(wp), co, ci, kh,
                                                      kw, cd, native.stream_ptr()),
                         "cn_pack_conv_weight")
            ev = torch.cuda.Event()
            ev.record()
            hit = (wp, factor, ev)
            if cacheable:
                self._wput(key, hit)
        self.keep += [hit[0], hit[1]]
        self._pack_events.append(hit[2])
        return (hit[0], hit[1]) if (f32s or prescale) else hit[0]

    @staticmethod
    def _narrow_form(kh, kw, padding, dilation, out_nchw, ci, co):
        return ci == 16 and co <= 32 and (kh, kw, padding, dilation) == (3, 3, 1, 1) and not out_nchw

    @classmethod
    def _f32s_conv_form(cls, kh, kw, stride, padding, dilation, out_nchw, ci=0, co=0):
        if cls._narrow_form(kh, kw, padding, dilation, out_nchw, ci, co):
            return stride == 1 and os.environ.get("CN_C16_F32S", "1") != "0"
        return True

    def _grow_ws(self, need):
        if need > self.ws_bytes:
            self.ws = torch.empty(need, device=self.device, dtype=torch.uint8)
            self.ws_bytes = need

    def set_input(self, C=3):
        self.input = Act(None, self.B, self.H, self.W, C, nchw=True, exp=self._exp("input"),
                         lid="input")
        return self.input

    def conv(self, x, weight, bias=None, bn=None, relu=False, residual=None, stride=1,
             padding=0, dilation=1, out_nchw=False, out=None, wsources=None, out_plain=False,
             pool=None, lid=None):
        co, ci, kh, kw = weight.shape
        assert ci == x.C, (ci, x.C)
        lid = self._lid(lid)
        Ho = _out_size(x.H, kh, stride, padding, dilation)
        Wo = _out_size(x.W, kw, stride, padding, dilation)
        use_s = self.split and not x.nchw and self._f32s_conv_form(kh, kw, stride, padding,
                                                                  dilation, out_nchw, ci, co)
        if use_s and self._narrow_form(kh, kw, padding, dilation, out_nchw, ci, co) and residual is None:
            x, out_plain = self.plain(x), True
        fuse_pool = False
        if pool is not None and tuple(pool) == (3, 2, 1) and self.split and x.nchw and out is None \
                and not out_nchw and residual is None and os.environ.get("CN_FUSE_STEM_POOL", "1") != "0":
            probe = ConvDesc(B=x.B, H=x.H, W=x.W, Cin=ci, Ho=Ho, Wo=Wo, Cout=co, KH=kh, KW=kw,
                             stride=stride, pad_h=padding, pad_w=padding, dil=dilation,
                             in_layout=LAYOUT_NCHW, out_layout=LAYOUT_NHWC, dtype=self.cdtype)
            fuse_pool = bool(self.lib.cn_stem_maxpool_supported(ctypes.byref(probe)))
        scale, shift = fold_bn(bias, bn, co, self.device)
        flags = 0
        stem_s = False
        if self.split and x.nchw and not use_s:
            probe = ConvDesc(B=x.B, H=x.H, W=x.W, Cin=ci, Ho=Ho, Wo=Wo, Cout=co, KH=kh, KW=kw,
                             stride=stride, pad_h=padding, pad_w=padding, dil=dilation,
                             in_layout=LAYOUT_NCHW, out_layout=LAYOUT_NHWC, dtype=self.cdtype,
                             OH=Ho, OW=Wo, oy_mul=1, ox_mul=1,
                             flags=CONV_STEM_F32S | (CONV_STEM_MAXPOOL if fuse_pool else 0))
            stem_s = bool(self.lib.cn_stem_f32s_supported(ctypes.byref(probe)))
        if use_s:
            wp, factor = self._pack(weight, wsources, f32s=True)
            if x.fmt == "f32":
                flags |= CONV_X_PLAIN
            if residual is not None and residual.fmt == "f32":
                flags |= CONV_R_PLAIN
            cd = DTYPE_F32S
        else:
            x, residual = self.plain(x), self.plain(residual)
            if stem_s:
                wp, factor = self._pack(weight, wsources, prescale=True)
                flags |= CONV_STEM_F32S
            else:
                wp, factor = self._pack(weight, wsources), None
            cd = self.cdtype
            if fuse_pool:
                flags |= CONV_STEM_MAXPOOL
        pool_lid = lid + "/pool" if pool is not None else None
        out_given = out is not None
        if out is None:
            if out_nchw:
                t = torch.empty((x.B, co, Ho, Wo), device=self.device, dtype=torch.float32)
                out = Act(t, x.B, Ho, Wo, co, nchw=True, lid=lid)
            elif fuse_pool:
                y_s = stem_s and co % 32 == 0 and os.environ.get("CN_STEM_Y_F32S", "1") != "0"
                out = self._new(x.B, Ho // 2, Wo // 2, co, fmt="f32s" if y_s else None, lid=pool_lid)
                if y_s:
                    flags |= CONV_STEM_Y_F32S
            else:
                out = self._new(x.B, Ho, Wo, co,
                                fmt="f32s" if (use_s and not out_plain) else None, lid=lid)
        else:
            out.lid, out.exp = lid, self._exp(lid)
        if use_s and out.fmt != "f32s":
            flags |= CONV_Y_PLAIN
        assert use_s or stem_s or out.fmt != "f32s"
        res_pitch = 0
        if residual is not None and residual.pitch != out.pitch:
            sliced = out.pitch != (out.C if out.fmt != "f32s" else (out.C + 31) // 32 * 32) or \
                residual.pitch != (residual.C if residual.fmt != "f32s" else (residual.C + 31) // 32 * 32)
            if sliced:
                res_pitch = residual.pitch
            else:
                assert use_s
                if out.fmt == "f32s":
                    residual = self.packed(residual)
                    flags &= ~CONV_R_PLAIN
                else:
                    residual = self.plain(residual)
                    flags |= CONV_R_PLAIN
                assert residual.pitch == out.pitch
        if res_pitch:
            probe = ConvDesc(B=x.B, H=x.H, W=x.W, Cin=ci, Ho=Ho, Wo=Wo, Cout=co, KH=kh, KW=kw,
                             stride=stride, pad_h=padding, pad_w=padding, dil=dilation,
                             in_layout=LAYOUT_NCHW if x.nchw else LAYOUT_NHWC, in_pitch=x.pitch,
                             out_layout=LAYOUT_NCHW if out.nchw else LAYOUT_NHWC, out_pitch=out.pitch,
                             OH=Ho, OW=Wo, oy_mul=1, oy_add=0, ox_mul=1, ox_add=0, relu=int(relu),
                             dtype=cd, flags=flags, res_pitch=res_pitch)
            if not self.lib.cn_conv2d_res_pitch_supported(ctypes.byref(probe)):
                assert out_given and residual.pitch == (residual.C if residual.fmt != "f32s"
                                                        else (residual.C + 31) // 32 * 32), \
                    "a residual slice needs a kernel that takes its pitch"
                return self.conv(x, weight, bias=bias, bn=bn, relu=relu, residual=residual, stride=stride,
                                 padding=padding, dilation=dilation, out_nchw=out_nchw, out=None,
                                 wsources=wsources, out_plain=out_plain, pool=pool, lid=lid)
        ctl = None
        if use_s or stem_s:
            ex, ey = x.exp, out.applied_exp
            k = factor * _pow2(ex - ey)
            scale = k if scale is None else scale * k
            if shift is not None:
                shift = shift * _pow2(-ey)
            res_mul = _pow2(residual.applied_exp - ey) if residual is not None else 1.0
            x_mul = _pow2(-ex) if (x.fmt == "f32" or x.nchw) else 1.0
            ctl = self._ctl(lid, x_mul, res_mul)
        scale = None if scale is None else scale.contiguous()
        shift = None if shift is None else shift.contiguous()
        self.keep += [scale, shift]
        d = ConvDesc(B=x.B, H=x.H, W=x.W, Cin=ci, Ho=Ho, Wo=Wo, Cout=co, KH=kh, KW=kw,
                     stride=stride, pad_h=padding, pad_w=padding, dil=dilation,
                     in_layout=LAYOUT_NCHW if x.nchw else LAYOUT_NHWC, in_pitch=x.pitch,
                     out_layout=LAYOUT_NCHW if out.nchw else LAYOUT_NHWC, out_pitch=out.pitch,
                     OH=Ho, OW=Wo, oy_mul=1, oy_add=0, ox_mul=1, ox_add=0, relu=int(relu),
                     dtype=cd, flags=flags)
        if ctl is not None:
            d.ctl = ctl
        if res_pitch:
            d.res_pitch = res_pitch
        fl = 2 * x.B * Ho * Wo * co * ci * kh * kw
        by = 4 * (x.B * x.H * x.W * ci + x.B * out.H * out.W * co * (2 if residual is not None else 1)
                  + co * ci * kh * kw)
        self._emit_conv(d, x, wp, scale, shift, residual, out, dict(kind="conv", flops=fl, bytes=by))
        self.flops += fl
        if pool is not None and not fuse_pool:
            return self.maxpool(out, *pool, lid=pool_lid)
        return out

    def _emit_conv(self, d, x, wp, scale, shift, residual, out, meta):
        lib = self.lib
        self.keep.append(d)
        is_input = x is self.input
        sp, hp = native.ptr(scale), native.ptr(shift)
        rp = residual.ptr() if residual is not None else None
        wpp, op = native.ptr(wp), out.ptr()
        dref = ctypes.byref(d)
        self._grow_ws(lib.cn_conv2d_workspace_bytes(dref))

        def run():
            xp = ctypes.c_void_p(self.input.t.data_ptr()) if is_input else x.ptr()
            wsp = ctypes.c_void_p(self.ws.data_ptr()) if self.ws is not None else None
            rc = lib.cn_conv2d(dref, xp, wpp, sp, hp, rp, op, wsp, self.ws_bytes,
                               native.stream_ptr())
            if rc:
                native.check(rc, "cn_conv2d")
        self.ops.append(run)
        self.meta.append(meta)
        self.trace.append((meta["kind"], out))

    def conv_transpose4x4s2(self, x, weight, bn=None, relu=False, out_plain=False):
        ci, co, kh, kw = weight.shape
        assert (kh, kw) == (4, 4) and ci == x.C
        assert self.dtype == torch.float32, "ConvTranspose is built for fp32 only"
        lib = self.lib
        lid = self._lid()
        use_s = self.split
        scale, shift = fold_bn(None, bn, co, self.device)
        cacheable = isinstance(weight, torch.nn.Parameter)
        key = self._wkey("deconv4x4s2_f32s" if use_s else "deconv4x4s2", [weight])
        hit = self.wcache.get(key) if cacheable else None
        if hit is None:
            w = weight.detach().to(device=self.device, dtype=torch.float32)
            factor = None
            if use_s:
                wt, factor = prescale_rows(w.transpose(0, 1).contiguous())
                w = wt.transpose(0, 1)
            w = w.contiguous()
            wp = torch.empty(lib.cn_packed_deconv4x4s2_weight_floats(ci, co), device=self.device,
                             dtype=torch.float32)
            native.check(lib.cn_pack_deconv4x4s2_weight(native.ptr(w), native.ptr(wp), ci, co,
                                                        DTYPE_F32S if use_s else DTYPE_F32,
                                                        native.stream_ptr()),
                         "cn_pack_deconv4x4s2_weight")
            ev = torch.cuda.Event()
            ev.record()
            hit = (wp, factor, ev)
            if cacheable:
                self._wput(key, hit)
        wp, factor, ev = hit
        self._pack_events.append(ev)
        flags = 0
        out = self._new(x.B, 2 * x.H, 2 * x.W, co, fmt="f32s" if (use_s and not out_plain) else None,
                        lid=lid)
        ctl = None
        if use_s:
            ey = out.applied_exp
            k = factor * _pow2(x.exp - ey)
            scale = (k if scale is None else scale * k).contiguous()
            if shift is not None:
                shift = (shift * _pow2(-ey)).contiguous()
            if x.fmt == "f32":
                flags |= CONV_X_PLAIN
            if out_plain:
                flags |= CONV_Y_PLAIN
            ctl = self._ctl(lid, _pow2(-x.exp) if x.fmt == "f32" else 1.0)
        self.keep += [scale, shift, wp, factor]
        sp, hp, wpp = native.ptr(scale), native.ptr(shift), native.ptr(wp)
        cd = DTYPE_F32S if use_s else DTYPE_F32
        cref = ctypes.byref(ctl) if ctl is not None else None

        def run():
            rc = lib.cn_conv_transpose4x4s2(x.ptr(), wpp, sp, hp, out.ptr(), x.B, x.H, x.W, ci, co,
                                            x.pitch, out.pitch, int(relu), cd, flags, cref,
                                            native.stream_ptr())
            if rc:
                native.check(rc, "cn_conv_transpose4x4s2")
        self.ops.append(run)
        fl = 2 * x.B * (2 * x.H) * (2 * x.W) * co * ci * 4
        by = 4 * (x.B * x.H * x.W * (ci + 4 * co) + co * ci * 16)
        self.meta.append(dict(kind="conv", flops=fl, bytes=by))
        self.trace.append(("deconv", out))
        self.flops += fl
        return out

    def maxpool(self, x, k, s, pad, lid=None, out=None, to_s=False):
        assert self.dtype == torch.float32, "max-pool is built for fp32 only"
        lid = self._lid(lid)
        lib = self.lib
        from_s = x.fmt == "f32s" and x.C % 32 == 0
        Ho, Wo = _out_size(x.H, k, s, pad), _out_size(x.W, k, s, pad)
        if from_s and (to_s or (out is not None and out.fmt == "f32s")):
            if out is None:
                out = self._new(x.B, Ho, Wo, x.C, fmt="f32s", lid=lid)
            else:
                assert out.fmt == "f32s" and (out.B, out.H, out.W, out.C) == (x.B, Ho, Wo, x.C)
                out.lid, out.exp = lid, self._exp(lid)
            assert x.c_off % 32 == 0 and out.c_off % 32 == 0
            mul = _pow2(x.exp - out.exp)
            ctl = self._ctl(lid)

            def run():
                rc = lib.cn_maxpool_nhwc_f32s(x.ptr(), out.ptr(), x.B, x.H, x.W, x.C, x.pitch, out.pitch,
                                              k, s, pad, mul, ctl.range, native.stream_ptr())
                if rc:
                    native.check(rc, "cn_maxpool_nhwc_f32s")
            self.ops.append(run)
            self.meta.append(dict(kind="maxpool", flops=0, bytes=4 * x.B * x.C * (x.H * x.W + Ho * Wo)))
            self.trace.append(("maxpool", out))
            return out
        if not from_s:
            x = self.plain(x)
        private = self._new(x.B, Ho, Wo, x.C, lid=lid)
        assert x.pitch == x.C and x.c_off == 0
        mul = _pow2(x.exp) if from_s else 1.0

        def run():
            rc = lib.cn_maxpool_nhwc_scaled(x.ptr(), private.ptr(), x.B, x.H, x.W, x.C, k, s, pad,
                                            DTYPE_F32S if from_s else DTYPE_F32, mul,
                                            native.stream_ptr())
            if rc:
                native.check(rc, "cn_maxpool_nhwc")
        self.ops.append(run)
        self.meta.append(dict(kind="maxpool", flops=0,
                              bytes=4 * x.B * x.C * (x.H * x.W + Ho * Wo)))
        self.trace.append(("maxpool", private))
        return private

    def _emit_simple(self, fn, kind, out, nbytes):
        self.ops.append(fn)
        self.meta.append(dict(kind=kind, flops=0, bytes=nbytes))
        self.trace.append((kind, out))

    def concat_buffer(self, B, H, W, widths):
        if not self.split or any(w % 32 for w in widths) or os.environ.get("CN_CONCAT_INPLACE", "1") == "0":
            return None, None
        C = sum(widths)
        buf = self._new(B, H, W, C, fmt="f32s")
        slices, off = [], 0
        for w in widths:
            slices.append(Act(buf.t, B, H, W, w, pitch=C, c_off=off, fmt="f32s"))
            off += w
        return buf, slices

    def concat(self, acts, into=None):
        lid = self._lid()
# ... 356 lines not shown
        builder.finish()
        self.b = builder
        self.outputs = outputs
        self.deferred = builder.deferred
        self.graph = None
        self._static_in = None

    @property
    def flops(self):
        return self.b.flops

    def run(self, images, events=None, event_after=None, borrow=False, digest=False):
        if not images.is_cuda:
            raise native.NativeError("input batch must be on a HIP device; there is no CPU path")
        native.require_f32(images)
        images = images.contiguous()
        assert tuple(images.shape) == (self.b.B, self.b.input.C, self.b.H, self.b.W), images.shape
        if self.b._pack_events:
            st = torch.cuda.current_stream()
            for ev in self.b._pack_events:
                st.wait_event(ev)
            self.b._pack_events = []
        if self.graph is not None:
            self._static_in.copy_(images)
            self.graph.replay()
        else:
            self.b.input.t = images
            if events is None:
                for op in self.b.ops:
                    op()
            else:
                e = torch.cuda.Event(enable_timing=True)
                e.record()
                events.append(e)
                for i, op in enumerate(self.b.ops):
                    op()
                    if event_after is None or i in event_after:
                        e = torch.cuda.Event(enable_timing=True)
                        e.record()
                        events.append(e)
        b = self.b
        if b.range is not None and b.range_slots:
            if digest:
                b.range_sum_host.copy_(b.range_sum, non_blocking=True)
                b.range_sum_event.record()
            self._digest_fresh = bool(digest)
        out = {k: (v.t if borrow else v.t.clone()) for k, v in self.outputs.items()}
        if self.deferred is not None:
            out["_deferred"] = self.deferred
        return out

    def range_report(self, reset=True):
        b = self.b
        if b.range is None or not b.range_slots:
            return None
        n = len(b.range_slots)
        RL = b.RANGE_LAUNCHES
        host = torch.cat([st[:, :min(RL, n - i * RL)] for i, (_, st) in enumerate(b.range_chunks)], dim=1).cpu()
        if reset:
            for _, st in b.range_chunks:
                st[0].zero_()
                st[1].fill_(0x7f800000)
        hi = host[0].contiguous().view(torch.float32).tolist()
        lo = host[1].contiguous().view(torch.float32).tolist()
        return [(lid, (hi[i][0], lo[i][0]), (hi[i][1], lo[i][1])) for i, lid in enumerate(b.range_slots)]

    def range_quick(self):
        b = self.b
        if b.range is None or not b.range_slots:
            return "ok"
        if getattr(self, "_digest_fresh", False):
            b.range_sum_event.synchronize()
            vals = b.range_sum_host.tolist()
        else:
            vals = b.range_sum.tolist()
        hi, lo = (int(v) & 0xffffffff for v in vals)
        if hi > F16_MAX_BITS:
            return "overflow"
        if getattr(self, "ignore_low", False):
            return "ok"
        return "low" if lo < LOW_WATER_BITS else "ok"

    def range_status(self, reset=True):
        if self.range_quick() == "ok":
            return "ok", []
        rep = self.range_report(reset)
        if reset and rep is not None:
            self.b.range_sum.copy_(torch.tensor([0, 0x7f800000], dtype=torch.int32))
            self.b.range_sum_host.copy_(torch.tensor([0, 0x7f800000], dtype=torch.int32))
        if rep is None:
            return "ok", []
        over = [r for r in rep if r[1][0] > F16_MAX or r[2][0] > F16_MAX or
                r[1][0] != r[1][0] or r[2][0] != r[2][0]]
        if over:
            return "overflow", over
        if getattr(self, "ignore_low", False):
            return "ok", []
        low = [r for r in rep if any(side[0] > 0.0 and side[1] < LOW_WATER for side in r[1:])]
        return ("low", low) if low else ("ok", [])

    def capture(self):
        self._static_in = torch.zeros((self.b.B, self.b.input.C, self.b.H, self.b.W),
                                      device=self.b.device, dtype=torch.float32)
        self.b.input.t = self._static_in
        s = torch.cuda.Stream()
        s.wait_stream(torch.cuda.current_stream())
        with torch.cuda.stream(s):
            for _ in range(2):
                for op in self.b.ops:
                    op()
        torch.cuda.current_stream().wait_stream(s)
        g = torch.cuda.CUDAGraph()
        with torch.cuda.graph(g):
            for op in self.b.ops:
                op()
        self.graph = g
        torch.cuda.current_stream().synchronize()
        self.b.range_reset()
        return self


class RangeError(native.NativeError):
    """An f32s forward clamped a value although it had just been calibrated on that very input."""


class PlannedModule(torch.nn.Module):

    def describe(self, pb, x):
        raise NotImplementedError

    compute_dtype = torch.float32
    f32s = None

    def fp32_mfma(self, enable=True):
        self.f32s = (not enable) if enable is not None else None
        self.drop_plans()
        return self

    def half_compute(self, enable=True):
        self.compute_dtype = torch.float16 if enable else torch.float32
        self.drop_plans()
        return self

    range_tracking_on = True

    def range_tracking(self, enable=True):
        self.range_tracking_on = bool(enable)
        self.drop_plans()
        return self

    def drop_plans(self):
        self.__dict__["_plans"] = {}

    def defer_heads(self, names=()):
        self.__dict__["_defer"] = tuple(names)
        return self

    def deferral(self):
        return self.__dict__.get("_defer", ())

    def deferred_names(self):
        if self.compute_dtype != torch.float32:
            return ()
        return self.deferral()

    max_plans = int(os.environ.get("CN_PLAN_CACHE", "8"))

    def uses_f32s(self):
        split = self.f32s if self.f32s is not None else os.environ.get("CN_F32S", "1") != "0"
        return bool(split) and self.compute_dtype == torch.float32

    @property
    def exponents(self):
        return self.__dict__.get("_exps")

    def calibrate(self, x, merge=False):
        if not x.is_cuda:
            raise native.NativeError("calibration needs a batch on a HIP device")
        B, C, H, W = x.shape
        lib = native.lib()
        with torch.no_grad():
            pb = PlanBuilder(x.device, B, H, W, dtype=torch.float32, wcache={}, calibrating=True)
            outs = self.describe(pb, pb.set_input(C))
            plan = Plan(pb, outs)
            plan.run(x.contiguous().float(), borrow=True)
            acts = [a for _, a in pb.trace if a is not None and a.lid is not None and not a.nchw]
            words = torch.zeros(len(acts) + 1, device=x.device, dtype=torch.int32)
            st = native.stream_ptr()
            xc = x.contiguous()
            native.check(lib.cn_absmax_f32(native.ptr(xc), xc.numel(), 1, 1, native.ptr(words), st),
                         "cn_absmax_f32")
            for i, a in enumerate(acts):
                wptr = ctypes.c_void_p(words.data_ptr() + 4 * (i + 1))
                native.check(lib.cn_absmax_f32(a.ptr(), a.B * a.H * a.W, a.C, a.pitch, wptr, st),
                             "cn_absmax_f32")
            vals = words.cpu().view(torch.float32).tolist()
        amax = {"input": vals[0]}
        for a, v in zip(acts, vals[1:]):
            amax[a.lid] = max(amax.get(a.lid, 0.0), v)
        exps = {lid: exponent_for(v) for lid, v in amax.items()}
        for grp in pb.groups:
            have = [exps[l] for l in grp if l in exps and amax.get(l, 0.0) > 0.0]
            if have:
                e = max(have)
                for l in grp:
                    exps[l] = e
        old = self.__dict__.get("_exps")
        if merge == "decay" and old:
            for l, e in old.items():
                exps[l] = max(exps.get(l, e), e - LOW_STEP)
        elif merge and old:
            for l, e in old.items():
                exps[l] = max(e, exps.get(l, e))
        self.__dict__["_absmax"] = amax
        self.__dict__["_calibrations"] = self.__dict__.get("_calibrations", 0) + 1
        if old is not None and exps == old:
            for plan in self.__dict__.get("_plans", {}).values():
                plan.ignore_low = True
            return exps
        self.__dict__["_exps"] = exps
        self.__dict__["_plans"] = {}
        return exps

    def plan_for(self, B, H, W, device, deferred=None):
        cache = self.__dict__.setdefault("_plans", {})
        defer = () if deferred is False else self.deferred_names()
        key = (B, H, W, str(device), self.compute_dtype, self.f32s, self.range_tracking_on, defer)
        plan = cache.pop(key, None)
        if plan is None:
            native.lib()
            with torch.no_grad():
                pb = PlanBuilder(device, B, H, W, dtype=self.compute_dtype,
                                 wcache=self.__dict__.setdefault("_wcache", {}), split=self.f32s,
                                 exps=self.__dict__.get("_exps"),
                                 track=None if self.range_tracking_on else False, defer=defer)
                x = pb.set_input(3)
                outs = self.describe(pb, x)
            plan = Plan(pb, outs)
            while len(cache) >= max(1, self.max_plans):
                cache.pop(next(iter(cache)))
        cache[key] = plan
        return plan

    def invalidate_plans(self):
        self.__dict__["_plans"] = {}
        self.__dict__["_wcache"] = {}
        self.__dict__["_exps"] = None

    def load_state_dict(self, *a, **kw):
        r = super().load_state_dict(*a, **kw)
        self.invalidate_plans()
        return r

    def _apply(self, fn, *a, **kw):
        r = super()._apply(fn, *a, **kw)
        self.invalidate_plans()
        return r

    def range_ok(self, x=None):
        worst = "ok"
        for plan in list(self.__dict__.get("_plans", {}).values()):
            st, bad = plan.range_status()
            if st == "overflow":
                worst = "overflow"
                self.__dict__["_last_range_event"] = ("overflow", bad)
            elif st == "low" and worst == "ok":
                worst = "low"
                self.__dict__["_last_range_event"] = ("low", bad)
        if worst == "overflow":
            if x is not None:
                self.calibrate(x, merge=True)
            else:
                self.__dict__["_recalibrate"] = "merge"
            return False
        if worst == "low":
            self._schedule_low()
        return True

    def _schedule_low(self):
        nf, at = self.__dict__.get("_nfwd", 0), self.__dict__.get("_low_cal_at")
        if at is not None and nf - at < LOW_EVERY:
            if not self.__dict__.get("_low_warned"):
                self.__dict__["_low_warned"] = True
                warnings.warn("f32s: activations keep falling below the calibrated range; "
                              "re-calibration is limited to once per %d forwards" % LOW_EVERY)
            return
        self.__dict__["_low_cal_at"] = nf
        self.__dict__["_recalibrate"] = "decay"

    def forward(self, x, borrow=False, events=None, event_after=None, check=None, deferred=False):
        if self.training:
            raise native.NativeError("centernet_amd implements the inference path only; call .eval()")
        if not x.is_cuda:
            raise native.NativeError(
                "centernet_amd runs on MI355X only (input is on %s). There is no CPU path: the "
                "CPU restatement under oracle/ is test infrastructure." % x.device)
        B, C, H, W = x.shape
        f32s = self.uses_f32s()
        if f32s:
            pending = self.__dict__.pop("_recalibrate", None)
            if self.__dict__.get("_exps") is None:
                self.calibrate(x)
            elif pending:
                self.calibrate(x, merge=True if pending == "merge" else pending)
            self.__dict__["_nfwd"] = self.__dict__.get("_nfwd", 0) + 1
        if check is None:
            check = f32s and not borrow
        deferred = bool(deferred)
        plan = self.plan_for(B, H, W, x.device, deferred)
        out = plan.run(x, events=events, event_after=event_after, borrow=borrow, digest=bool(check and f32s))
        if check and f32s:
            st, bad = plan.range_status()
            if st == "overflow":
                self.calibrate(x, merge=True)
                plan = self.plan_for(B, H, W, x.device, deferred)
                if events is not None:
                    del events[:]
                out = plan.run(x, events=events, event_after=event_after, borrow=borrow)
                st, bad = plan.range_status()
                if st == "overflow":
                    raise RangeError("f32s forward still clamps after re-calibration: %r" % (bad[:3],))
            elif st == "low":
                self._schedule_low()
        return [out]
```

centernet_amd/native.py:

```python
import contextlib
import ctypes
import os
import subprocess

import numpy as np
import torch

_HERE = os.path.dirname(os.path.abspath(__file__))
LIB_PATH = os.environ.get("CENTERNET_AMD_LIB") or os.path.join(_HERE, "libcenternet_amd.so")
CSRC = os.path.join(_HERE, "csrc")

CN_OK = 0
LAYOUT_NCHW = 0
LAYOUT_NHWC = 1
DTYPE_F32 = 0
DTYPE_F16 = 1
DTYPE_F32S = 2
CONV_X_PLAIN, CONV_Y_PLAIN, CONV_R_PLAIN, CONV_STEM_F32S, CONV_STEM_MAXPOOL = 1, 2, 4, 8, 16
CONV_STEM_Y_F32S = 32
MERGE_MAX_ROWS = 2048
MERGE_MAX_CLASSES = 1024
DECODE_SIGMOID = 1
DECODE_DDD_RAW_DEPTH = 16384

IMAGE_DESC = np.dtype([("offset", np.uint64), ("H", np.int32), ("W", np.int32), ("pitch", np.int32),
                       ("reserved", np.int32), ("dst_to_src", np.float64, (6,)), ("scale", np.float64, (2,))])
assert IMAGE_DESC.itemsize == 88

_lib = None


class NativeError(RuntimeError):
    pass


class F32sCtl(ctypes.Structure):
    _fields_ = [("x_mul", ctypes.c_float), ("res_mul", ctypes.c_float), ("range", ctypes.c_void_p)]


class ConvDesc(ctypes.Structure):
    _fields_ = [(n, ctypes.c_int) for n in (
        "B", "H", "W", "Cin", "Ho", "Wo", "Cout", "KH", "KW", "stride", "pad_h", "pad_w",
        "dil", "in_layout", "in_pitch", "out_layout", "out_pitch", "OH", "OW", "oy_mul",
        "oy_add", "ox_mul", "ox_add", "relu", "dtype", "flags", "res_pitch")] + [("ctl", F32sCtl)]


class HeadOut(ctypes.Structure):
    _fields_ = [("w", ctypes.c_void_p), ("bias", ctypes.c_void_p), ("y", ctypes.c_void_p),
                ("cout", ctypes.c_int), ("reserved", ctypes.c_int), ("oscale", ctypes.c_void_p),
                ("w_frag", ctypes.c_void_p)]


def build(force=False, verbose=False):
    args = ["make", "-C", CSRC, "-j8"]
    if force:
        args.append("-B")
    out = None if verbose else subprocess.DEVNULL
    subprocess.check_call(args, stdout=out)
    if not os.path.exists(LIB_PATH):
        raise NativeError("build did not produce %s" % LIB_PATH)
    return LIB_PATH


def _declare(lib):
    vp, i, sz = ctypes.c_void_p, ctypes.c_int, ctypes.c_size_t
    lib.cn_version.restype = i
    lib.cn_status_string.restype = ctypes.c_char_p
    lib.cn_status_string.argtypes = [i]
    lib.cn_arch.restype = ctypes.c_char_p
    lib.cn_set_tuning.restype = i
    lib.cn_set_tuning.argtypes = [i, i]
    lib.cn_get_tuning.restype = i
    lib.cn_get_tuning.argtypes = [i, ctypes.POINTER(i)]
    lib.cn_reset_tuning.restype = i
    lib.cn_dcn_v2_forward_workspace_bytes.restype = sz
    lib.cn_dcn_v2_forward_workspace_bytes.argtypes = [i] * 8
    lib.cn_dcn_v2_forward_f32.restype = i
    lib.cn_dcn_v2_forward_f32.argtypes = [vp] * 6 + [i] * 15 + [vp, sz, vp]
    lib.cn_dcn_v2_forward_nhwc_f32.restype = i
    lib.cn_dcn_v2_forward_nhwc_f32.argtypes = [vp, vp, vp, vp, i, vp, vp, vp] + [i] * 7 + [vp, sz, vp]
    lib.cn_dcn_v2_forward_nhwc_workspace_bytes.restype = sz
    lib.cn_dcn_v2_forward_nhwc_workspace_bytes.argtypes = [i] * 5
    lib.cn_f32_to_f32s.restype = i
    lib.cn_f32_to_f32s.argtypes = [vp, vp, sz, i, i, i, vp]
    lib.cn_f32s_to_f32.restype = i
    lib.cn_f32s_to_f32.argtypes = [vp, vp, sz, i, i, i, vp]
    f = ctypes.c_float
    ctl = ctypes.POINTER(F32sCtl)
    lib.cn_f32_to_f32s_scaled.restype = i
    lib.cn_f32_to_f32s_scaled.argtypes = [vp, vp, sz, i, i, i, f, vp, vp]
    lib.cn_f32s_to_f32_scaled.restype = i
    lib.cn_f32s_to_f32_scaled.argtypes = [vp, vp, sz, i, i, i, f, vp]
    lib.cn_absmax_f32.restype = i
    lib.cn_absmax_f32.argtypes = [vp, sz, i, i, vp, vp]
    lib.cn_range_fold.restype = i
    lib.cn_range_fold.argtypes = [vp, vp, vp, i, vp]
    lib.cn_range_fold_digest.restype = i
    lib.cn_range_fold_digest.argtypes = [vp, vp, vp, vp, i, vp]
    lib.cn_packed_head_w2_bytes.restype = sz
    lib.cn_packed_head_w2_bytes.argtypes = [i]
    lib.cn_pack_head_w2_f32s.restype = i
    lib.cn_pack_head_w2_f32s.argtypes = [vp, vp, i, vp]
    lib.cn_flip_average_f32.restype = i
    lib.cn_flip_average_f32.argtypes = [vp, vp, i, i, i, vp, vp, i, vp]
    lib.cn_flip_average_f32_batch.restype = i
    lib.cn_flip_average_f32_batch.argtypes = [vp, vp, i, i, i, i, vp, vp, i, i, vp]
    lib.cn_calib_mfma_f16.restype = ctypes.c_double
    lib.cn_calib_mfma_f16.argtypes = [vp, i, vp]
    lib.cn_calib_copy.restype = i
    lib.cn_calib_copy.argtypes = [vp, vp, sz, vp]
    lib.cn_calib_clock.restype = i
    lib.cn_calib_clock.argtypes = [vp, i, vp]
    lib.cn_calib_latency.restype = i
    lib.cn_calib_latency.argtypes = [vp, ctypes.c_uint32, i, vp, vp, vp]
    lib.cn_maxpool_nhwc_f32s.restype = i
    lib.cn_maxpool_nhwc_f32s.argtypes = [vp, vp, i, i, i, i, i, i, i, i, i, f, vp, vp]
    lib.cn_maxpool_nhwc_scaled.restype = i
    lib.cn_maxpool_nhwc_scaled.argtypes = [vp, vp, i, i, i, i, i, i, i, i, f, vp]
    lib.cn_dcn_v2_forward_nhwc.restype = i
    lib.cn_dcn_v2_forward_nhwc.argtypes = [vp, vp, vp, vp, i, vp, vp, vp] + [i] * 10 + [ctl, vp, sz, vp]
    lib.cn_pack_deconv4x4s2_weight.restype = i
    lib.cn_pack_deconv4x4s2_weight.argtypes = [vp, vp, i, i, i, vp]
    lib.cn_conv_transpose4x4s2.restype = i
    lib.cn_conv_transpose4x4s2.argtypes = [vp, vp, vp, vp, vp] + [i] * 10 + [ctl, vp]
    lib.cn_heads3x3_1x1.restype = i
    lib.cn_heads3x3_1x1.argtypes = [vp, i, i, i, i, i, vp, vp, vp, i, i, vp, i, i, ctl, vp]
    lib.cn_packed_conv_weight_floats.restype = sz
    lib.cn_packed_conv_weight_floats.argtypes = [i] * 4
    lib.cn_pack_conv_weight_f32.restype = i
    lib.cn_pack_conv_weight_f32.argtypes = [vp, vp, i, i, i, i, vp]
    lib.cn_stem_maxpool_supported.restype = i
    lib.cn_stem_maxpool_supported.argtypes = [ctypes.POINTER(ConvDesc)]
    lib.cn_stem_f32s_supported.restype = i
    lib.cn_stem_f32s_supported.argtypes = [ctypes.POINTER(ConvDesc)]
    lib.cn_conv2d_f32.restype = i
    lib.cn_conv2d_f32.argtypes = [ctypes.POINTER(ConvDesc), vp, vp, vp, vp, vp, vp, vp]
    lib.cn_packed_conv_weight_elems.restype = sz
    lib.cn_packed_conv_weight_elems.argtypes = [i] * 5
    lib.cn_pack_conv_weight.restype = i
    lib.cn_pack_conv_weight.argtypes = [vp, vp, i, i, i, i, i, vp]
    lib.cn_conv2d_res_pitch_supported.restype = i
    lib.cn_conv2d_res_pitch_supported.argtypes = [ctypes.POINTER(ConvDesc)]
    lib.cn_conv2d_workspace_bytes.restype = sz
    lib.cn_conv2d_workspace_bytes.argtypes = [ctypes.POINTER(ConvDesc)]
    lib.cn_conv2d.restype = i
    lib.cn_conv2d.argtypes = [ctypes.POINTER(ConvDesc), vp, vp, vp, vp, vp, vp, vp, sz, vp]
    lib.cn_upsample2x_add_f16.restype = i
    lib.cn_upsample2x_add_f16.argtypes = [vp, vp, vp, i, i, i, i, vp]
    lib.cn_packed_deconv4x4s2_weight_floats.restype = sz
    lib.cn_packed_deconv4x4s2_weight_floats.argtypes = [i, i]
    lib.cn_pack_deconv4x4s2_weight_f32.restype = i
    lib.cn_pack_deconv4x4s2_weight_f32.argtypes = [vp, vp, i, i, vp]
    lib.cn_conv_transpose4x4s2_f32.restype = i
    lib.cn_conv_transpose4x4s2_f32.argtypes = [vp] * 5 + [i] * 8 + [vp]
    lib.cn_maxpool3x3s2_nhwc_f32.restype = i
    lib.cn_maxpool3x3s2_nhwc_f32.argtypes = [vp, vp, i, i, i, i, vp]
    lib.cn_maxpool_nhwc_f32.restype = i
    lib.cn_maxpool_nhwc_f32.argtypes = [vp, vp, i, i, i, i, i, i, i, vp]
    lib.cn_maxpool_nhwc.restype = i
    lib.cn_maxpool_nhwc.argtypes = [vp, vp, i, i, i, i, i, i, i, i, vp]
    lib.cn_dw_conv_transpose_f32.restype = i
    lib.cn_dw_conv_transpose_f32.argtypes = [vp, vp, vp, vp, i, i, i, i, i, vp]
    lib.cn_copy_channels_f32.restype = i
    lib.cn_copy_channels_f32.argtypes = [vp, i, vp, i, sz, i, vp]
    lib.cn_upsample2x_add_f32.restype = i
    lib.cn_upsample2x_add_f32.argtypes = [vp, vp, vp, i, i, i, i, vp]
    lib.cn_heads3x3_1x1_f32.restype = i
    lib.cn_heads3x3_1x1_f32.argtypes = [vp, i, i, i, i, i, vp, vp, i, i, ctypes.POINTER(HeadOut), vp]
    lib.cn_warp_normalize_u8_f32.restype = i
    lib.cn_warp_normalize_u8_f32.argtypes = [vp, i, i, i, ctypes.POINTER(ctypes.c_double), i, i,
                                             ctypes.POINTER(ctypes.c_float),
                                             ctypes.POINTER(ctypes.c_float), i, vp, vp]
    lib.cn_warp_normalize_u8_f32_batch.restype = i
    lib.cn_warp_normalize_u8_f32_batch.argtypes = [vp, i, sz, i, i, i, ctypes.POINTER(ctypes.c_double), i, i,
                                                   ctypes.POINTER(ctypes.c_float), ctypes.POINTER(ctypes.c_float),
                                                   i, vp, vp]
    lib.cn_warp_normalize_u8_f32_ragged.restype = i
    lib.cn_warp_normalize_u8_f32_ragged.argtypes = [vp, vp, i, i, i, ctypes.POINTER(ctypes.c_float),
                                                    ctypes.POINTER(ctypes.c_float), i, vp, vp]
    lib.cn_resize_bilinear_u8_ragged.restype = i
    lib.cn_resize_bilinear_u8_ragged.argtypes = [vp, vp, vp, vp, i, i, i, vp]
    lib.cn_warp_table_u8_f32_batch.restype = i
    lib.cn_warp_table_u8_f32_batch.argtypes = [vp, i, sz, i, i, i, ctypes.POINTER(ctypes.c_double), i, i, vp, vp, vp]
    lib.cn_warp_table_u8_f32_ragged.restype = i
    lib.cn_warp_table_u8_f32_ragged.argtypes = [vp, vp, i, i, i, vp, vp, vp]
    lib.cn_ddd_post_process_f32.restype = i
    lib.cn_ddd_post_process_f32.argtypes = [vp, i, i, i, i, vp, i, vp, ctypes.c_float, vp, vp, vp, vp]
    lib.cn_ctdet_post_process_f32.restype = i
    lib.cn_ctdet_post_process_f32.argtypes = [vp, i, i, i, vp, i, ctypes.c_float, vp, vp, vp]
    lib.cn_ctdet_merge_f32.restype = i
    lib.cn_ctdet_merge_f32.argtypes = [vp, vp, i, i, i, i, i, i, vp, vp, vp]
    lib.cn_exdet_post_process_f32.restype = i
    lib.cn_exdet_post_process_f32.argtypes = [vp, i, i, i, i, vp, i, ctypes.c_float, vp, vp, vp]
    lib.cn_exdet_merge_f32.restype = i
    lib.cn_exdet_merge_f32.argtypes = [vp, vp, i, i, i, i, i, vp, vp, vp, vp]
    lib.cn_multi_pose_post_process_f32.restype = i
    lib.cn_multi_pose_post_process_f32.argtypes = [vp, i, i, vp, i, ctypes.c_float, vp, vp]
    lib.cn_multi_pose_merge_f32.restype = i
    lib.cn_multi_pose_merge_f32.argtypes = [vp, i, i, i, i, vp, vp]
    lib.cn_resize_bilinear_u8.restype = i
    lib.cn_resize_bilinear_u8.argtypes = [vp, i, i, i, i, i, vp, vp]
    lib.cn_warp_affine_u8_host.restype = i
    lib.cn_warp_affine_u8_host.argtypes = [vp, i, i, i, ctypes.POINTER(ctypes.c_double), i, i, vp]
    lib.cn_resize_linear_u8_host.restype = i
    lib.cn_resize_linear_u8_host.argtypes = [vp, i, i, i, i, i, vp]
    lib.cn_normalize_u8_chw_f32_host.restype = i
    lib.cn_normalize_u8_chw_f32_host.argtypes = [vp, i, i, vp, vp, vp]
    lib.cn_soft_nms_f32.restype = i
    lib.cn_soft_nms_f32.argtypes = [vp, i, i, ctypes.c_float, ctypes.c_float, ctypes.c_float, i]
    lib.cn_nchw_to_nhwc_f32.restype = i
    lib.cn_nchw_to_nhwc_f32.argtypes = [vp, vp, i, i, i, i, i, vp]
    lib.cn_nhwc_to_nchw_f32.restype = i
    lib.cn_nhwc_to_nchw_f32.argtypes = [vp, vp, i, i, i, i, i, vp]
    lib.cn_ctdet_decode_workspace_bytes.restype = sz
    lib.cn_ctdet_decode_workspace_bytes.argtypes = [i] * 5
    lib.cn_decode_state_region.restype = i
    lib.cn_decode_state_region.argtypes = [i] * 5 + [ctypes.POINTER(ctypes.c_size_t)] * 2
    lib.cn_ctdet_decode_f32.restype = i
    lib.cn_ctdet_decode_f32.argtypes = [vp, vp, vp] + [i] * 7 + [vp, vp, vp, sz, vp]
    lib.cn_nms_topk_channel_f32.restype = i
    lib.cn_nms_topk_channel_f32.argtypes = [vp] + [i] * 6 + [vp, vp, vp, sz, vp]
    lib.cn_topk_f32.restype = i
    lib.cn_topk_f32.argtypes = [vp] + [i] * 6 + [vp, vp, vp, vp, sz, vp]
    lib.cn_pack_cell_heads_w1.restype = i
    lib.cn_pack_cell_heads_w1.argtypes = [vp, vp, i, i, vp]
    lib.cn_ctdet_heads_at_cells_f32.restype = i
    lib.cn_ctdet_heads_at_cells_f32.argtypes = [vp, i, i, i, i, i, i, ctypes.c_float, vp, vp, vp, i, vp, vp, i, i,
                                                vp, vp, vp, vp, vp]
    lib.cn_gather_feat_f32.restype = i
    lib.cn_gather_feat_f32.argtypes = [vp, vp, vp] + [i] * 5 + [vp]
    lib.cn_ddd_decode_workspace_bytes.restype = sz
    lib.cn_ddd_decode_workspace_bytes.argtypes = [i] * 5
    lib.cn_ddd_decode_f32.restype = i
    lib.cn_ddd_decode_f32.argtypes = [vp] * 6 + [i] * 6 + [vp, vp, sz, vp]
    lib.cn_exct_decode_workspace_bytes.restype = sz
    lib.cn_exct_decode_workspace_bytes.argtypes = [i] * 5
    lib.cn_exct_aggregate_f32.restype = i
    lib.cn_exct_aggregate_f32.argtypes = [vp, vp, i, i, i, i, i, ctypes.c_float, vp]
    lib.cn_exct_decode_f32.restype = i
    lib.cn_exct_decode_f32.argtypes = [vp] * 9 + [i] * 5 + [ctypes.c_float, ctypes.c_float, i, i,
                                                        vp, vp, sz, vp]
    lib.cn_agnex_ct_decode_workspace_bytes.restype = sz
    lib.cn_agnex_ct_decode_workspace_bytes.argtypes = [i] * 5
    lib.cn_agnex_ct_decode_f32.restype = i
    lib.cn_agnex_ct_decode_f32.argtypes = [vp] * 9 + [i] * 5 + [ctypes.c_float, ctypes.c_float, i, i,
                                                            vp, vp, sz, vp]
    lib.cn_multi_pose_decode_workspace_bytes.restype = sz
    lib.cn_multi_pose_decode_workspace_bytes.argtypes = [i] * 6
    lib.cn_multi_pose_decode_f32.restype = i
    lib.cn_multi_pose_decode_f32.argtypes = [vp] * 6 + [i] * 7 + [vp, vp, sz, vp]


def lib():
    global _lib
    if _lib is None:
        if not os.path.exists(LIB_PATH):
            raise NativeError(
                "%s is missing: build it with `make -C %s` (hipcc, gfx950). "
                "centernet_amd has no CPU or PyTorch fallback." % (LIB_PATH, CSRC))
        l = ctypes.CDLL(LIB_PATH)
        _declare(l)
        _lib = l
    return _lib


def check(rc, what):
    if rc != CN_OK:
        raise NativeError("%s failed: %s (%d)" % (what, lib().cn_status_string(rc).decode(), rc))


@contextlib.contextmanager
def tuning(knobs):
    l = lib()
    before = {}
    for key in knobs:
        v = ctypes.c_int()
        check(l.cn_get_tuning(key, ctypes.byref(v)), "cn_get_tuning(%d)" % key)
        before[key] = v.value
    try:
        for key, value in knobs.items():
            check(l.cn_set_tuning(key, value), "cn_set_tuning(%d, %d)" % (key, value))
        yield
    finally:
        for key, value in before.items():
            l.cn_set_tuning(key, value)


def stream_ptr():
    return ctypes.c_void_p(torch.cuda.current_stream().cuda_stream)


def ptr(t):
    if t is None:
        return None
    if not t.is_cuda:
# ... 12 lines not shown
```

centernet_amd/networks/resnet.py:

```python
import torch.nn as nn

from ..dcn_v2 import DCN
from ..engine import PlannedModule
from .common import bn, conv, bilinear_upsample_init_, detection_head


class BasicBlock(nn.Module):
    expansion = 1

    def __init__(self, inplanes, planes, stride=1, downsample=None):
        super().__init__()
        self.stride, self.downsample = stride, downsample
        self.conv1, self.bn1 = conv(inplanes, planes, 3, stride), bn(planes)
        self.conv2, self.bn2 = conv(planes, planes, 3), bn(planes)

    def describe(self, pb, x, out_plain=False):
        res = x
        if self.downsample is not None:
            ds = self.downsample
            res = pb.conv(x, ds[0].weight, bn=ds[1], stride=ds[0].stride[0])
        out = pb.conv(x, self.conv1.weight, bn=self.bn1, relu=True, stride=self.stride, padding=1)
        return pb.conv(out, self.conv2.weight, bn=self.bn2, relu=True, residual=res, padding=1,
                       out_plain=out_plain)


class Bottleneck(nn.Module):
    expansion = 4

    def __init__(self, inplanes, planes, stride=1, downsample=None):
        super().__init__()
        wide = planes * self.expansion
        self.stride, self.downsample = stride, downsample
        self.conv1, self.bn1 = conv(inplanes, planes, 1), bn(planes)
        self.conv2, self.bn2 = conv(planes, planes, 3, stride), bn(planes)
        self.conv3, self.bn3 = conv(planes, wide, 1), bn(wide)

    def describe(self, pb, x, out_plain=False):
        res = x
        if self.downsample is not None:
            ds = self.downsample
            res = pb.conv(x, ds[0].weight, bn=ds[1], stride=ds[0].stride[0])
        out = pb.conv(x, self.conv1.weight, bn=self.bn1, relu=True)
        out = pb.conv(out, self.conv2.weight, bn=self.bn2, relu=True, stride=self.stride, padding=1)
        return pb.conv(out, self.conv3.weight, bn=self.bn3, relu=True, residual=res,
                       out_plain=out_plain)


class PoseResNet(PlannedModule):
    STAGE_WIDTHS = (64, 128, 256, 512)

    def __init__(self, block, layers, heads, head_conv, dcn=True):
        super().__init__()
        self.heads, self.use_dcn = heads, dcn
        self.deconv_with_bias = False
        self.conv1, self.bn1 = conv(3, 64, 7, 2), bn(64)
        self.relu, self.maxpool = nn.ReLU(inplace=True), nn.MaxPool2d(3, 2, 1)
        width = 64
        for stage, (planes, count) in enumerate(zip(self.STAGE_WIDTHS, layers), start=1):
            blocks, width = self._stage(block, width, planes, count, stride=1 if stage == 1 else 2)
            setattr(self, 'layer%d' % stage, blocks)
        up_widths = (256, 128, 64) if dcn else (256, 256, 256)
        self.deconv_layers = self._up_path(width, up_widths)
        for name in (heads if dcn else sorted(heads)):
            setattr(self, name, detection_head(up_widths[-1], head_conv, heads[name],
                                               is_heatmap='hm' in name, normal_init=dcn))

    @staticmethod
    def _stage(block, width_in, planes, count, stride):
        width_out = planes * block.expansion
        project = None
        if stride != 1 or width_in != width_out:
            project = nn.Sequential(conv(width_in, width_out, 1, stride), bn(width_out))
        blocks = [block(width_in, planes, stride, project)]
        blocks += [block(width_out, planes) for _ in range(count - 1)]
        return nn.Sequential(*blocks), width_out

    def _up_path(self, width, up_widths):
        mods = []
        for planes in up_widths:
            if self.use_dcn:
                mods += [DCN(width, planes, kernel_size=(3, 3), stride=1, padding=1, dilation=1,
                             deformable_groups=1), bn(planes), nn.ReLU(inplace=True)]
                width = planes
            up = nn.ConvTranspose2d(width, planes, 4, 2, 1, 0, bias=self.deconv_with_bias)
            if self.use_dcn:
                bilinear_upsample_init_(up)
            mods += [up, bn(planes), nn.ReLU(inplace=True)]
            width = planes
        return nn.Sequential(*mods)

    def describe(self, pb, x):
        x = pb.conv(x, self.conv1.weight, bn=self.bn1, relu=True, stride=2, padding=3,
                    pool=(self.maxpool.kernel_size, self.maxpool.stride, self.maxpool.padding))
        mods = list(self.deconv_layers)
        blocks = [blk for layer in (self.layer1, self.layer2, self.layer3, self.layer4) for blk in layer]
        for blk in blocks:
            x = blk.describe(pb, x, out_plain=blk is blocks[-1] and bool(mods) and isinstance(mods[0], DCN))
        i = 0
        while i < len(mods):
            m = mods[i]
            if isinstance(m, DCN):
                x = pb.dcn(x, m, bn=mods[i + 1], relu=True)
                i += 3
            elif isinstance(m, nn.ConvTranspose2d):
                to_dcn = i + 3 < len(mods) and isinstance(mods[i + 3], DCN)
                x = pb.conv_transpose4x4s2(x, m.weight, bn=mods[i + 1], relu=True, out_plain=to_dcn)
                i += 3
            else:
                raise RuntimeError("unexpected module in deconv_layers: %r" % m)
        return pb.heads(x, {h: getattr(self, h) for h in self.heads})


resnet_spec = {18: (BasicBlock, [2, 2, 2, 2]),
               34: (BasicBlock, [3, 4, 6, 3]),
               50: (Bottleneck, [3, 4, 6, 3]),
               101: (Bottleneck, [3, 4, 23, 3]),
               152: (Bottleneck, [3, 8, 36, 3])}


def get_pose_net_dcn(num_layers, heads, head_conv=256):
    block, layers = resnet_spec[num_layers]
    return PoseResNet(block, layers, heads, head_conv=head_conv, dcn=True)


def get_pose_net(num_layers, heads, head_conv):
    block, layers = resnet_spec[num_layers]
    return PoseResNet(block, layers, heads, head_conv=head_conv, dcn=False)
```

include/centernet_amd.h:

```cpp
#ifndef CENTERNET_AMD_H
#define CENTERNET_AMD_H

#include <stddef.h>
#include <stdint.h>

#ifdef __cplusplus
extern "C" {
#endif

typedef enum cn_status {
    CN_OK = 0,
    CN_ERR_SHAPE = -1,
    CN_ERR_UNSUPPORTED = -2,
    CN_ERR_WORKSPACE = -3,
    CN_ERR_LAUNCH = -4,
    CN_ERR_NULL = -5,
    CN_ERR_ALIGN = -6
} cn_status;

#define CN_LAYOUT_NCHW 0
#define CN_LAYOUT_NHWC 1

#define CN_DTYPE_F32 0
#define CN_DTYPE_F16 1
#define CN_DTYPE_F32S 2

#define CN_RANGE_SLOTS 64
#define CN_RANGE_STRIDE 16
#define CN_RANGE_WORDS (2 * CN_RANGE_SLOTS * CN_RANGE_STRIDE)
typedef struct cn_f32s_ctl {
    float x_mul;
    float res_mul;
    uint32_t *range;
} cn_f32s_ctl;

int cn_version(void);
const char *cn_status_string(int status);
const char *cn_arch(void);
int cn_set_tuning(int key, int value);
int cn_get_tuning(int key, int *value);
int cn_reset_tuning(void);



size_t cn_dcn_v2_forward_workspace_bytes(int B, int Cin, int H, int W, int Cout,
                                         int kernel_h, int kernel_w, int layout);

int cn_dcn_v2_forward_f32(const float *input, const float *weight, const float *bias,
                          const float *offset, const float *mask, float *output,
                          int B, int Cin, int H, int W, int Cout,
                          int kernel_h, int kernel_w, int stride_h, int stride_w,
                          int pad_h, int pad_w, int dilation_h, int dilation_w,
                          int deformable_group, int apply_mask_sigmoid,
                          void *workspace, size_t workspace_bytes, void *stream);

size_t cn_dcn_v2_forward_nhwc_workspace_bytes(int B, int Cin, int H, int W, int Cout);
int cn_dcn_v2_forward_nhwc(const float *input_nhwc, const void *weight_packed, const float *bias,
                           const float *offset_mask_nhwc, int om_pitch, const float *scale,
                           const float *shift, void *output_nhwc, int out_pitch, int B, int Cin,
                           int H, int W, int Cout, int mask_sigmoid, int relu, int dtype, int flags,
                           const cn_f32s_ctl *ctl, void *workspace, size_t workspace_bytes,
                           void *stream);
int cn_dcn_v2_forward_nhwc_f32(const float *input_nhwc, const float *weight_packed,
                               const float *bias, const float *offset_mask_nhwc,
                               int om_pitch, const float *scale, const float *shift,
                               float *output_nhwc, int B, int Cin, int H, int W,
                               int Cout, int mask_sigmoid, int relu, void *workspace,
                               size_t workspace_bytes, void *stream);

int cn_f32_to_f32s(const float *x, void *y, size_t npix, int C, int in_pitch, int out_pitch,
                   void *stream);
int cn_f32s_to_f32(const void *x, float *y, size_t npix, int C, int in_pitch, int out_pitch,
                   void *stream);
int cn_f32_to_f32s_scaled(const float *x, void *y, size_t npix, int C, int in_pitch, int out_pitch,
                          float mul, uint32_t *range, void *stream);
int cn_f32s_to_f32_scaled(const void *x, float *y, size_t npix, int C, int in_pitch, int out_pitch,
                          float mul, void *stream);
int cn_absmax_f32(const float *x, size_t npix, int C, int pitch, uint32_t *word, void *stream);
int cn_range_fold(uint32_t *cur, uint32_t *hi, uint32_t *lo, int n_launches, void *stream);
int cn_range_fold_digest(uint32_t *cur, uint32_t *hi, uint32_t *lo, uint32_t *summary,
                         int n_launches, void *stream);

int cn_flip_average_f32(float *x_pair, float *out, int C, int H, int W, const int32_t *chan_src,
                        const float *chan_sign, int apply_sigmoid, void *stream);
int cn_flip_average_f32_batch(float *x_pairs, float *out, int P, int C, int H, int W, const int32_t *chan_src,
                              const float *chan_sign, int apply_sigmoid, int mode, void *stream);
double cn_calib_mfma_f16(float *sink, int iters, void *stream);
int cn_calib_copy(const void *src, void *dst, size_t bytes, void *stream);
int cn_calib_latency(const uint32_t *chain, uint32_t start, int steps, uint32_t *atom,
                     unsigned long long *out, void *stream);
int cn_calib_clock(unsigned long long *out, int ticks, void *stream);

typedef struct cn_conv_desc {
    int B, H, W, Cin;
    int Ho, Wo, Cout;
    int KH, KW;
    int stride, pad_h, pad_w, dil;
    int in_layout, in_pitch;
    int out_layout, out_pitch;
    int OH, OW, oy_mul, oy_add, ox_mul, ox_add;
    int relu;
    int dtype;
    int flags;
    int res_pitch;
    cn_f32s_ctl ctl;
} cn_conv_desc;
int cn_conv2d_res_pitch_supported(const cn_conv_desc *d);
#define CN_CONV_X_PLAIN 1
#define CN_CONV_Y_PLAIN 2
#define CN_CONV_R_PLAIN 4
#define CN_CONV_STEM_F32S 8
#define CN_CONV_STEM_MAXPOOL 16
#define CN_CONV_STEM_Y_F32S 32

int cn_stem_maxpool_supported(const cn_conv_desc *d);
int cn_stem_f32s_supported(const cn_conv_desc *d);

size_t cn_packed_conv_weight_floats(int Cout, int Cin, int KH, int KW);
int cn_pack_conv_weight_f32(const float *w_oihw, float *w_packed, int Cout, int Cin,
                            int KH, int KW, void *stream);

int cn_conv2d_f32(const cn_conv_desc *desc, const float *x, const float *w_packed,
                  const float *scale, const float *shift, const float *residual,
                  float *y, void *stream);
size_t cn_packed_conv_weight_elems(int Cout, int Cin, int KH, int KW, int dtype);
int cn_pack_conv_weight(const float *w_oihw, void *w_packed, int Cout, int Cin, int KH, int KW,
                        int dtype, void *stream);
size_t cn_conv2d_workspace_bytes(const cn_conv_desc *desc);
int cn_conv2d(const cn_conv_desc *desc, const void *x, const void *w_packed, const float *scale,
              const float *shift, const void *residual, void *y, void *workspace,
              size_t workspace_bytes, void *stream);

size_t cn_packed_deconv4x4s2_weight_floats(int Cin, int Cout);
int cn_pack_deconv4x4s2_weight(const float *w_iohw, void *w_packed, int Cin, int Cout, int dtype,
                               void *stream);
int cn_conv_transpose4x4s2(const void *x_nhwc, const void *w_packed, const float *scale,
                           const float *shift, void *y_nhwc, int B, int H, int W, int Cin, int Cout,
                           int in_pitch, int out_pitch, int relu, int dtype, int flags,
                           const cn_f32s_ctl *ctl, void *stream);
int cn_pack_deconv4x4s2_weight_f32(const float *w_iohw, float *w_packed, int Cin, int Cout,
                                   void *stream);
int cn_conv_transpose4x4s2_f32(const float *x_nhwc, const float *w_packed, const float *scale,
                               const float *shift, float *y_nhwc, int B, int H, int W, int Cin,
                               int Cout, int in_pitch, int out_pitch, int relu, void *stream);

int cn_maxpool3x3s2_nhwc_f32(const float *x, float *y, int B, int H, int W, int C,
                             void *stream);
int cn_maxpool_nhwc_f32(const float *x, float *y, int B, int H, int W, int C, int k,
                        int s, int pad, void *stream);
int cn_maxpool_nhwc(const void *x_nhwc, float *y_nhwc, int B, int H, int W, int C, int k, int s,
                    int pad, int in_dtype, void *stream);
int cn_maxpool_nhwc_scaled(const void *x_nhwc, float *y_nhwc, int B, int H, int W, int C, int k,
                           int s, int pad, int in_dtype, float out_mul, void *stream);
int cn_maxpool_nhwc_f32s(const void *x, void *y, int B, int H, int W, int C, int in_pitch, int out_pitch,
                         int k, int s, int pad, float mul, uint32_t *range, void *stream);

int cn_dw_conv_transpose_f32(const float *x, const float *w_taps, const float *add, float *y,
                             int B, int H, int W, int C, int f, void *stream);
int cn_copy_channels_f32(const float *src, int src_pitch, float *dst, int dst_pitch,
                         size_t npix, int C, void *stream);
int cn_upsample2x_add_f32(const float *x, const float *add, float *y, int B, int H, int W,
                          int C, void *stream);
int cn_upsample2x_add_f16(const void *x, const void *add, void *y, int B, int H, int W, int C,
                          void *stream);

typedef struct cn_head_out {
    const float *w;
    const float *bias;
    float *y;
    int cout;
    int reserved;
    const float *oscale;
    const void *w_frag;
} cn_head_out;
size_t cn_packed_head_w2_bytes(int cout);
int cn_pack_head_w2_f32s(const float *w, void *out, int cout, void *stream);
int cn_heads3x3_1x1_f32(const float *x, int B, int H, int W, int Cin, int in_pitch,
                        const float *w1_packed, const float *bias1, int head_conv, int n_heads,
                        const cn_head_out *heads, void *stream);
int cn_heads3x3_1x1(const void *x, int B, int H, int W, int Cin, int in_pitch,
                    const void *w1_packed, const float *scale1, const float *bias1, int head_conv,
                    int n_heads, const cn_head_out *heads, int dtype, int flags,
                    const cn_f32s_ctl *ctl, void *stream);

int cn_warp_normalize_u8_f32(const uint8_t *image_hwc, int H, int W, int pitch_bytes,
                             const double *dst_to_src_2x3, int out_h, int out_w,
                             const float *mean3, const float *std3, int flip_concat,
                             float *out_nchw, void *stream);
int cn_warp_normalize_u8_f32_batch(const uint8_t *images_hwc, int N, size_t image_stride_bytes, int H, int W,
                                   int pitch_bytes, const double *dst_to_src_2x3, int out_h, int out_w,
                                   const float *mean3, const float *std3, int flip_concat,
                                   float *out_nchw, void *stream);
typedef struct cn_image_desc {
    uint64_t offset;
    int32_t H, W, pitch;
    int32_t reserved;
    double dst_to_src[6];
    double scale_x, scale_y;
} cn_image_desc;
int cn_warp_normalize_u8_f32_ragged(const uint8_t *packed, const cn_image_desc *descs_dev, int N, int out_h,
                                    int out_w, const float *mean3, const float *std3, int flip_concat,
                                    float *out_nchw, void *stream);
int cn_resize_bilinear_u8_ragged(const uint8_t *packed_in, const cn_image_desc *in_descs_dev, uint8_t *packed_out,
                                 const cn_image_desc *out_descs_dev, int N, int max_out_h, int max_out_w,
                                 void *stream);
int cn_ctdet_post_process_f32(const float *dets, int B, int K, int num_classes, const double *to_source_2x3,
                              int per_image, float scale, float *rows, int32_t *bounds, void *stream);
#define CN_MERGE_MAX_ROWS 2048
#define CN_MERGE_MAX_CLASSES 1024
int cn_ctdet_merge_f32(const float *rows, const int32_t *bounds, int S, int B, int K, int num_classes,
                       int apply_nms, int max_per_image, float *out_rows, int32_t *out_bounds, void *stream);
int cn_exdet_post_process_f32(const float *dets, int B, int R, int num_classes, int out_width,
                              const double *to_source_2x3, int per_image, float scale, float *rows,
                              int32_t *bounds, void *stream);
int cn_exdet_merge_f32(const float *rows, const int32_t *bounds, int S, int B, int R, int num_classes,
                       int max_per_image, float *out_rows, int32_t *out_bounds, int32_t *status, void *stream);
int cn_multi_pose_post_process_f32(const float *dets, int B, int K, const double *to_source_2x3, int per_image,
                                   float scale, float *rows, void *stream);
int cn_multi_pose_merge_f32(const float *rows, int S, int B, int K, int apply_nms, float *out_rows,
                            void *stream);
int cn_resize_bilinear_u8(const uint8_t *image_hwc, int H, int W, int pitch_bytes, int out_h,
                          int out_w, uint8_t *out_hwc, void *stream);

int cn_warp_table_u8_f32_batch(const uint8_t *images_hwc, int N, size_t image_stride_bytes, int H, int W,
                               int pitch_bytes, const double *dst_to_src_2x3, int out_h, int out_w,
                               const float *table_3x256, float *out_nchw, void *stream);
int cn_warp_table_u8_f32_ragged(const uint8_t *packed, const cn_image_desc *descs_dev, int N, int out_h,
                                int out_w, const float *table_3x256, float *out_nchw, void *stream);
int cn_ddd_post_process_f32(const float *dets, int B, int K, int row_floats, int num_classes,
                            const double *to_source_2x3, int per_image, const float *calibs, float peak_thresh,
                            float *rows, int32_t *bounds, int32_t *kept, void *stream);

int cn_warp_affine_u8_host(const uint8_t *image_hwc, int h_in, int w_in, int channels,
                           const double *dst_to_src_2x3, int h_out, int w_out, uint8_t *out_hwc);
int cn_resize_linear_u8_host(const uint8_t *image_hwc, int h_in, int w_in, int channels, int h_out,
                             int w_out, uint8_t *out_hwc);

int cn_normalize_u8_chw_f32_host(const uint8_t *image_hwc, int h, int w, const float *mean3,
                                 const float *std3, float *out_chw);

int cn_soft_nms_f32(float *boxes_host, int n, int stride, float sigma, float Nt,
                    float threshold, int method);

int cn_nchw_to_nhwc_f32(const float *x, float *y, int B, int C, int H, int W,
                        int out_pitch, void *stream);
int cn_nhwc_to_nchw_f32(const float *x, float *y, int B, int C, int H, int W,
                        int in_pitch, void *stream);

size_t cn_ctdet_decode_workspace_bytes(int B, int C, int H, int W, int K);

int cn_ctdet_decode_f32(const float *heat, const float *wh, const float *reg,
                        int B, int C, int H, int W, int K, int cat_spec_wh,
                        int apply_sigmoid, float *dets, int32_t *inds,
                        void *workspace, size_t workspace_bytes, void *stream);

#define CN_DECODE_SIGMOID 1
#define CN_DECODE_NO_PEAK_TEST 512
#define CN_DECODE_STATE_CLEAN 4096
int cn_decode_state_region(int B, int C, int H, int W, int K, size_t *offset, size_t *bytes);
// ... 59 lines not shown
```

Measured before the change: 12310 img/s.

## Fuse downsample 1x1 projection into the second 3x3 conv of ResNet blocks

```diff
diff --git a/centernet_amd/csrc/cn_conv.hip b/centernet_amd/csrc/cn_conv.hip
--- a/centernet_amd/csrc/cn_conv.hip
+++ b/centernet_amd/csrc/cn_conv.hip
@@ -1026,6 +1026,18 @@
     return dense_ksplit(d, a) > 1 ? 0 : 1;
 }
 
+static bool proj_form_ok(const cn_conv_desc *d, bool planning)
+{
+    IgemmArgs a = {};
+    if (!d || conv_fill_args(d, &a) != CN_OK) return false;
+    if (d->dtype != CN_DTYPE_F32S || !is_3x3s1(d) || d->in_layout != CN_LAYOUT_NHWC ||
+        d->out_layout != CN_LAYOUT_NHWC || (d->flags & ~CN_CONV_Y_PLAIN))
+        return false;
+    if (planning && cn_knobs.nohalo) return false;
+    return cn_conv3x3p_proj_takes(d->B, d->H, d->W, d->Cin, d->Cout, d->in_pitch, d->out_pitch, false, &d->proj, planning);
+}
+extern "C" int cn_conv2d_proj_supported(const cn_conv_desc *d) { return proj_form_ok(d, true) ? 1 : 0; }
+
 extern "C" size_t cn_conv2d_workspace_bytes(const cn_conv_desc *d)
 {
     IgemmArgs a = {};
@@ -1050,6 +1062,14 @@
         if (d->in_layout == CN_LAYOUT_NHWC && !(d->flags & CN_CONV_X_PLAIN) && !aligned128(x)) return CN_ERR_ALIGN;
         if (d->out_layout == CN_LAYOUT_NHWC && !(d->flags & CN_CONV_Y_PLAIN) && !aligned128(y)) return CN_ERR_ALIGN;
         if (residual && !(d->flags & CN_CONV_R_PLAIN) && !aligned128(residual)) return CN_ERR_ALIGN;
+    }
+    if (d->proj.x) {
+        if (!d->proj.w || !scale) return CN_ERR_NULL;
+        if (residual || !proj_form_ok(d, false)) return CN_ERR_UNSUPPORTED;
+        if (!aligned128(d->proj.x) || !cn_aligned16(d->proj.w) || !cn_aligned16(y)) return CN_ERR_ALIGN;
+        return cn_conv3x3s1_persist(x, w_packed, scale, shift, nullptr, y, d->B, d->H, d->W, d->Cin, d->Cout, d->in_pitch,
+                                    d->out_pitch, d->out_pitch, d->relu, (d->flags & CN_CONV_Y_PLAIN) ? 1 : 0, 0, &d->ctl,
+                                    (hipStream_t)stream, &d->proj);
     }
     const bool f16 = (d->dtype == CN_DTYPE_F16);
     const size_t valign = f16 ? 8 : 16;
diff --git a/centernet_amd/csrc/cn_conv3x3p.hip b/centernet_amd/csrc/cn_conv3x3p.hip
--- a/centernet_amd/csrc/cn_conv3x3p.hip
+++ b/centernet_amd/csrc/cn_conv3x3p.hip
@@ -48,6 +48,11 @@
     float res_mul;
     uint32_t *range;
     int stagger;
+    const char *px;
+    const char *pw;
+    int pHi, pWi, ppitchB;
+    int pcinB;
+    int pnchunk;
     int knobs;
     int dbg;
     unsigned long long *prof;
@@ -108,9 +113,12 @@
 constexpr int p3_halo_loaders(int ntap, bool s2) { return (P3_HALO2 && (s2 || ntap == 4)) ? 2 : 1; }
 constexpr int p3_threads(int ntap, bool s2) { return 320 + 64 * p3_halo_loaders(ntap, s2); }
 
-template <int RES, bool OUT_PLAIN, bool DBG = false, bool HEADS = false, int NTAP = 9, bool S2 = false, bool PIPE = false>
+template <int RES, bool OUT_PLAIN, bool DBG = false, bool HEADS = false, int NTAP = 9, bool S2 = false, bool PIPE = false,
+          bool PROJ = false>
 __global__ __launch_bounds__(p3_threads(NTAP, S2), 4) void conv3x3p_kernel(const P3Args a, const P3Heads hd)
 {
+    static_assert(!PROJ || (PIPE && RES == 0 && !DBG && !HEADS && NTAP == 9 && !S2),
+                  "projection: the pipelined nine-tap stride-1 form without a residual");
     static_assert(!PIPE || !DBG, "pipelined fragment schedule: not in the instrumented instantiation");
     static_assert(!S2 || (NTAP == 9 && RES == 0 && !DBG && !HEADS), "stride 2: nine taps, no residual");
     constexpr int RES_AT = 0;
@@ -145,16 +153,56 @@
 #define P3_IC(v) std::integral_constant<int, (v)>{}
         if (wave == 4) {
             unsigned wofs[8];
+            unsigned wpofs[PROJ ? 8 : 1];
             auto set_wofs = [&](int nb) {
 #pragma unroll
                 for (int p = 0; p < 8; ++p) {
                     const int n = 8 * p + prow;
                     const int row = min(nb * 64 + n, a.cout_pad - 1);
                     wofs[p] = (unsigned)(row * a.cin_padB + ((ps ^ ((n >> 1) & 7)) << 4));
+                    if constexpr (PROJ) wpofs[p] = (unsigned)(row * a.pcinB + ((ps ^ ((n >> 1) & 7)) << 4));
                 }
             };
             set_wofs(first % a.nblk);
             const size_t tapB = (size_t)a.cout_pad * a.cin_padB;
+            if constexpr (PROJ) {
+                const int nst = a.nchunk + a.pnchunk;
+                int wk = 0, wc = 0, wt = 0, wg = 0;
+                auto issue_W = [&]() {
+                    if (wk >= nit) return;
+                    char *dst = smem + P_WOFF + (wg & (P_NSLOT - 1)) * P_WSLOT;
+                    if (wc < a.nchunk) {
+                        const char *base = a.w + (size_t)wt * tapB + (size_t)wc * 128;
+#pragma unroll
+                        for (int p = 0; p < 8; ++p)
+                            __builtin_amdgcn_global_load_lds((p3_gl_void *)(base + wofs[p]), (p3_lds_void *)(dst + p * 1024), 16, 0, 0);
+                        if (++wt < NTAP) { ++wg; return; }
+                        wt = 0;
+                    } else {
+                        const char *base = a.pw + (size_t)(wc - a.nchunk) * 128;
+#pragma unroll
+                        for (int p = 0; p < 8; ++p)
+                            __builtin_amdgcn_global_load_lds((p3_gl_void *)(base + wpofs[p]), (p3_lds_void *)(dst + p * 1024), 16, 0, 0);
+                    }
+                    ++wg;
+                    if (++wc == nst) {
+                        wc = 0;
+                        ++wk;
+                        if (wk < nit && a.nblk > 1) set_wofs((first + wk * nx) % a.nblk);
+                    }
+                };
+                issue_W();
+                issue_W();
+                issue_W();
+                const int T = nit * (NTAP * a.nchunk + a.pnchunk);
+                for (int gs = 0;; ++gs) {
+                    if (gs >= T - 2) asm volatile("s_waitcnt vmcnt(0)" ::: "memory");
+                    else asm volatile("s_waitcnt vmcnt(16)" ::: "memory");
+                    p3_barrier();
+                    if (gs == T) break;
+                    issue_W();
+                }
+            } else {
             int wk = 0, wc = 0, wt = 0, wg = 0;
             size_t wpar = DECONV ? (size_t)((first / a.nblk) % a.npar) * NTAP * tapB : 0;
             auto issue_W = [&]() {
@@ -194,6 +242,7 @@
                     issue_W();
                 }
                 if (s == S) break;
+            }
             }
         } else {
             auto halo_loader = [&](auto HW) {
@@ -222,6 +271,13 @@
                     hbase = a.x + ((size_t)(hit.b * a.Hi + 2 * hit.ty0 + hp) * a.Wi + 2 * hit.tx0 + hq) * a.in_pitchB +
                             (size_t)hc * 128;
                 } else {
+                    if constexpr (PROJ) {
+                        if (hc >= a.nchunk) {
+                            hbase = a.px + ((size_t)(hit.b * a.pHi + 2 * hit.ty0) * a.pWi + 2 * hit.tx0) * a.ppitchB +
+                                    (size_t)(hc - a.nchunk) * 128;
+                            return;
+                        }
+                    }
                     hbase = a.x + ((size_t)(hit.b * a.Hi + hit.ty0) * a.Wi + hit.tx0) * a.in_pitchB + (size_t)hc * 128;
                 }
             };
@@ -248,7 +304,7 @@
                     return;
                 }
                 hj = 0;
-                if (++hc == a.nchunk) {
+                if (++hc == a.nchunk + (PROJ ? a.pnchunk : 0)) {
                     hc = 0;
                     ++hk;
                     if (hk < nit) hit = p3_decode(a, first + hk * nx);
@@ -257,7 +313,65 @@
             };
             issue_H(P3_IC(0), P3_IC(P_HP), 0);
             advance_H();
-            if constexpr (S2) {
+            if constexpr (PROJ) {
+                auto issue_P = [&](auto K0, auto K1, int buf) {
+                    constexpr int k0 = decltype(K0)::value, k1 = decltype(K1)::value;
+                    static_assert(8 * k1 <= P_HR, "pieces of the 8 x 16 tile: rows of the halo image");
+                    char *dst = smem + buf * P_HBYTES;
+#pragma unroll
+                    for (int k = k0; k < k1; ++k) {
+                        int yx = pyx[k];
+                        asm volatile("" : "+v"(yx));
+                        const int hy = yx & 255, hx = yx >> 8;
+                        const int iy = 2 * (hit.ty0 + hy), ix = 2 * (hit.tx0 + hx);
+                        const bool ok = hy < P_TH && hx < P_TW && iy < a.pHi && ix < a.pWi;
+                        const int off = 2 * (hy * a.pWi + hx) * a.ppitchB + ((ps ^ ((hx >> 1) & 7)) << 4);
+                        const char *src = ok ? hbase + off : zero;
+                        __builtin_amdgcn_global_load_lds((p3_gl_void *)src, (p3_lds_void *)(dst + k * 1024), 16, 0, 0);
+                    }
+                };
+                constexpr int NPP = ((P_TH - 1) * P_HW + P_TW + 7) / 8;
+                const int nst = a.nchunk + a.pnchunk;
+                int s = 0;
+                for (int k = 0; k < nit; ++k) {
+                    for (int c = 0; c < nst; ++c, ++s) {
+                        const bool lastst = (k == nit - 1 && c == nst - 1);
+                        const int nbuf = (s + 1) & 1;
+                        const bool nproj = (hc >= a.nchunk);
+                        if (c < a.nchunk) {
+#pragma unroll
+                            for (int t = 0; t < NTAP; ++t) {
+                                if (t == 0) asm volatile("s_waitcnt vmcnt(0)" ::: "memory");
+                                p3_barrier();
+                                if (nproj) {
+                                    if (t == 1) issue_P(P3_IC(0), P3_IC(3), nbuf);
+                                    if (t == 2) issue_P(P3_IC(3), P3_IC(6), nbuf);
+                                    if (t == 3) issue_P(P3_IC(6), P3_IC(9), nbuf);
+                                    if (t == 4) issue_P(P3_IC(9), P3_IC(12), nbuf);
+                                    if (t == 5) issue_P(P3_IC(12), P3_IC(15), nbuf);
+                                    if (t == 6) issue_P(P3_IC(15), P3_IC(NPP), nbuf);
+                                } else {
+                                    if (t == 1) issue_H(P3_IC(0), P3_IC(4), nbuf);
+                                    if (t == 2) issue_H(P3_IC(4), P3_IC(8), nbuf);
+                                    if (t == 3) issue_H(P3_IC(8), P3_IC(12), nbuf);
+                                    if (t == 4) issue_H(P3_IC(12), P3_IC(16), nbuf);
+                                    if (t == 5) issue_H(P3_IC(16), P3_IC(20), nbuf);
+                                    if (t == 6) issue_H(P3_IC(20), P3_IC(P_HP), nbuf);
+                                }
+                            }
+                        } else {
+                            asm volatile("s_waitcnt vmcnt(0)" ::: "memory");
+                            p3_barrier();
+                            if (!lastst) {
+                                if (nproj) issue_P(P3_IC(0), P3_IC(NPP), nbuf);
+                                else issue_H(P3_IC(0), P3_IC(P_HP), nbuf);
+                            }
+                        }
+                        if (!lastst) advance_H();
+                    }
+                }
+                p3_barrier();
+            } else if constexpr (S2) {
                 const int ST = 4 * S;
                 bool done = false;
                 auto run_stage = [&](auto N, int s) {
@@ -935,13 +1049,13 @@
             __builtin_amdgcn_sched_barrier(0);
             load_half(P3_IC(0), P3_IC(0), S2 ? 0 : (s & 1) * P_HBYTES, P_WOFF + (g & 3) * P_WSLOT, F0);
             __builtin_amdgcn_sched_barrier(0);
-            for (c = 0; c < a.nchunk; ++c, ++s) {
+            auto run_stage = [&](auto PJ, const int c, const bool more) {
                 const int hb0 = (s & 1) * P_HBYTES, hb1 = ((s + 1) & 1) * P_HBYTES;
                 auto HB = [&](int i) { return S2 ? p3_s2_buf(i) * P_HBYTES : hb0; };
                 auto WB = [&](int i) { return P_WOFF + ((g + i) & 3) * P_WSLOT; };
-                const bool more = (c + 1 < a.nchunk);
-                auto pstep = [&](auto T) {
+                auto pstep_ = [&](auto T, auto END) {
                     constexpr int t = decltype(T)::value;
+                    constexpr bool end = decltype(END)::value;
                     __builtin_amdgcn_sched_barrier(0);
                     __builtin_amdgcn_s_setprio(1);
                     mfma_front(F0);
@@ -956,29 +1070,41 @@
                     __builtin_amdgcn_s_setprio(0);
                     p3_lds_fence();
                     p3_barrier();
-                    if constexpr (t + 1 < NTAP) {
+                    if constexpr (!end) {
                         load_half(P3_IC(t + 1), P3_IC(0), HB(t + 1), WB(t + 1), F0);
                     } else {
-                        if (more) load_half(P3_IC(0), P3_IC(0), S2 ? 0 : hb1, WB(NTAP), F0);
+                        if (more) load_half(P3_IC(0), P3_IC(0), S2 ? 0 : hb1, WB(t + 1), F0);
                     }
                     __builtin_amdgcn_sched_barrier(0);
                     keep(F1);
                     mfma_back(F1);
                     __builtin_amdgcn_sched_barrier(0);
                 };
-                pstep(P3_IC(0));
-                pstep(P3_IC(1));
-                pstep(P3_IC(2));
-                if (c == 0) *reinterpret_cast<float *>(smem + P_SSOFF + wave * 256 + lane * 4) = ssv;
-                pstep(P3_IC(3));
-                if constexpr (!DECONV) {
-                    pstep(P3_IC(4));
-                    pstep(P3_IC(5));
-                    pstep(P3_IC(6));
-                    pstep(P3_IC(7));
-                    pstep(P3_IC(8));
-                }
-                g += NTAP;
+                auto pstep = [&](auto T) { pstep_(T, std::integral_constant<bool, decltype(T)::value + 1 == NTAP>{}); };
+                if constexpr (decltype(PJ)::value) {
+                    pstep_(P3_IC(0), std::true_type{});
+                    g += 1;
+                } else {
+                    pstep(P3_IC(0));
+                    pstep(P3_IC(1));
+                    pstep(P3_IC(2));
+                    if (c == 0) *reinterpret_cast<float *>(smem + P_SSOFF + wave * 256 + lane * 4) = ssv;
+                    pstep(P3_IC(3));
+                    if constexpr (!DECONV) {
+                        pstep(P3_IC(4));
+                        pstep(P3_IC(5));
+                        pstep(P3_IC(6));
+                        pstep(P3_IC(7));
+                        pstep(P3_IC(8));
+                    }
+                    g += NTAP;
+                }
+                ++s;
+            };
+            for (c = 0; c < a.nchunk; ++c) run_stage(std::false_type{}, c, PROJ || c + 1 < a.nchunk);
+            if constexpr (PROJ) {
+#pragma unroll 1
+                for (int j = 0; j < a.pnchunk; ++j) run_stage(std::true_type{}, a.nchunk + j, j + 1 < a.pnchunk);
             }
             if constexpr (RES != 0) {
                 __builtin_amdgcn_sched_barrier(0);
@@ -1076,6 +1202,19 @@
     if (cn_knobs.c3p < 2 && items < 256) return false;
     if ((long)B * H * W * (long)max(in_pitch, max(out_pitch, res_pitch)) * 4 >= (1L << 31)) return false;
     (void)Cin;
+    return true;
+}
+
+bool cn_conv3x3p_proj_takes(int B, int H, int W, int Cin, int Cout, int in_pitch, int out_pitch, bool in_plain,
+                            const cn_conv_proj *pj, bool planning)
+{
+    if (!pj || in_plain) return false;
+    if (planning && !cn_conv3x3p_takes(B, H, W, Cin, Cout, in_pitch, out_pitch, 0, in_plain, false)) return false;
+    if ((in_pitch & 31) || (out_pitch & 31) || (Cout % 32) || Cin < 1) return false;
+    if ((long)B * H * W * (long)max(in_pitch, out_pitch) * 4 >= (1L << 31)) return false;
+    if (pj->Cin < 32 || (pj->Cin & 31) || (pj->pitch & 31) || pj->pitch < pj->Cin) return false;
+    if (pj->H < 1 || pj->W < 1 || (pj->H - 1) / 2 + 1 != H || (pj->W - 1) / 2 + 1 != W) return false;
+    if ((long)B * pj->H * pj->W * (long)pj->pitch * 4 >= (1L << 31)) return false;
     return true;
 }
 
@@ -1219,7 +1358,7 @@
 int cn_conv3x3s1_persist(const void *x, const void *w_packed, const float *scale, const float *shift,
                          const void *residual, void *y, int B, int H, int W, int Cin, int Cout,
                          int in_pitch, int out_pitch, int res_pitch, int relu, int out_plain, int res_plain,
-                         const cn_f32s_ctl *ctl, hipStream_t st)
+                         const cn_f32s_ctl *ctl, hipStream_t st, const cn_conv_proj *proj)
 {
     P3Args a = {};
     a.x = (const char *)x; a.w = (const char *)w_packed; a.scale = scale; a.shift = shift;
@@ -1251,10 +1390,26 @@
         CN_SET_MAX_LDS_ONCE((conv3x3p_kernel<R, OP, false, false, 9, false, PIPE>), P_LDS);                       \
         hipLaunchKernelGGL((conv3x3p_kernel<R, OP, false, false, 9, false, PIPE>), grid, block, P_LDS, st, a, P3Heads{}); \
     } while (0)
+#define P3_LAUNCH_PROJ(OP)                                                                                       \
+    do {                                                                                                         \
+        CN_SET_MAX_LDS_ONCE((conv3x3p_kernel<0, OP, false, false, 9, false, true, true>), P_LDS);                 \
+        hipLaunchKernelGGL((conv3x3p_kernel<0, OP, false, false, 9, false, true, true>), grid, block, P_LDS, st, a, P3Heads{}); \
+    } while (0)
 #define P3_LAUNCH(R, OP)                                                    \
     do {                                                                    \
         if (a.knobs & 2) P3_LAUNCH_(R, OP, true); else P3_LAUNCH_(R, OP, false); \
     } while (0)
+    if (proj) {
+        if (residual) return CN_ERR_UNSUPPORTED;
+        a.px = (const char *)proj->x; a.pw = (const char *)proj->w;
+        a.pHi = proj->H; a.pWi = proj->W; a.ppitchB = proj->pitch * 4;
+        a.pcinB = proj->Cin * 4;
+        a.pnchunk = proj->Cin / 32;
+        a.knobs |= 2;
+        if (out_plain) P3_LAUNCH_PROJ(true); else P3_LAUNCH_PROJ(false);
+        CN_CHECK_LAUNCH();
+        return CN_OK;
+    }
     const int rmode = !residual ? 0 : (res_plain ? 2 : 1);
     if ((p3_probe_dbg || p3_probe_prof) && !out_plain && rmode < 2) {
         a.dbg = p3_probe_dbg;
@@ -1276,6 +1431,7 @@
     }
 #undef P3_LAUNCH
 #undef P3_LAUNCH_
+#undef P3_LAUNCH_PROJ
     CN_CHECK_LAUNCH();
     return CN_OK;
 }
diff --git a/centernet_amd/csrc/cn_internal.h b/centernet_amd/csrc/cn_internal.h
--- a/centernet_amd/csrc/cn_internal.h
+++ b/centernet_amd/csrc/cn_internal.h
@@ -66,7 +66,9 @@
 int cn_conv3x3s1_persist(const void *x, const void *w_packed, const float *scale, const float *shift,
                          const void *residual, void *y, int B, int H, int W, int Cin, int Cout,
                          int in_pitch, int out_pitch, int res_pitch, int relu, int out_plain, int res_plain,
-                         const cn_f32s_ctl *ctl, hipStream_t st);
+                         const cn_f32s_ctl *ctl, hipStream_t st, const cn_conv_proj *proj = nullptr);
+bool cn_conv3x3p_proj_takes(int B, int H, int W, int Cin, int Cout, int in_pitch, int out_pitch, bool in_plain,
+                            const cn_conv_proj *pj, bool planning);
 bool cn_conv3x3s2p_takes(int B, int Hi, int Wi, int Cin, int Cout, int in_pitch, int out_pitch);
 int cn_conv3x3s2_persist(const void *x, const void *w_packed, const float *scale, const float *shift, void *y,
                          int B, int Hi, int Wi, int Cin, int Cout, int in_pitch, int out_pitch, int relu,
diff --git a/centernet_amd/engine.py b/centernet_amd/engine.py
--- a/centernet_amd/engine.py
+++ b/centernet_amd/engine.py
@@ -74,6 +74,43 @@
 
 def _pow2(e):
     return math.ldexp(1.0, int(e))
+
+
+PROJ_W_MIN = 1.0
+PROJ_MAX_BUMP = 8
+
+
+def fuse_projection_weights(w2, sc2, sh2, wp, scp, shp, e_mid, e_in):
+    w2 = w2.detach().float()
+    co = int(w2.shape[0])
+    wp = wp.detach().float().reshape(co, -1)
+    if sc2 is None or scp is None:
+        return None
+    sc2, scp = sc2.detach().float().to(w2.device), scp.detach().float().to(w2.device)
+    if not bool(torch.isfinite(sc2).all()) or bool((sc2 == 0).any()):
+        return None
+    ratio = scp / sc2
+    if not bool(torch.isfinite(ratio).all()):
+        return None
+    _, factor = prescale_rows(w2)
+    e_w2 = torch.frexp(factor)[1] - 1
+    shiftby = (int(e_in) - int(e_mid)) - e_w2
+    stored = torch.ldexp(wp * ratio[:, None], shiftby[:, None].expand_as(wp))
+    if not bool(torch.isfinite(stored).all()):
+        return None
+    top = stored.abs().amax(dim=1)
+    bump = (torch.frexp(top)[1] - 16).clamp_min(0)
+    bump = bump + (torch.ldexp(top, -bump) > F16_MAX).to(bump.dtype)
+    if int(bump.max()) > PROJ_MAX_BUMP:
+        return None
+    stored = torch.ldexp(stored, (-bump)[:, None].expand_as(stored))
+    top = torch.ldexp(top, -bump)
+    if float(top.max()) > F16_MAX or bool(((top > 0) & (top < PROJ_W_MIN)).any()):
+        return None
+    shift = torch.zeros(co, device=w2.device) if sh2 is None else sh2.detach().float().to(w2.device)
+    if shp is not None:
+        shift = shift + shp.detach().float().to(w2.device)
+    return stored.contiguous(), shift.contiguous(), bump.to(torch.int32)
 
 
 def pack_cell_heads(firsts, lasts, device):
@@ -122,9 +159,10 @@
     RANGE_WORDS = 2 * 64 * 16
 
     def __init__(self, device, B, H, W, dtype=torch.float32, wcache=None, split=None, exps=None,
-                 calibrating=False, track=None, defer=()):
+                 calibrating=False, track=None, defer=(), fuse_proj=True):
         assert dtype in (torch.float32, torch.float16)
         self.device = device
+        self.fuse_proj = bool(fuse_proj)
         self.defer = () if calibrating else tuple(defer)
         self.deferred = None
         if split is None:
@@ -279,6 +317,71 @@
         self._pack_events.append(hit[2])
         return (hit[0], hit[1]) if (f32s or prescale) else hit[0]
 
+    def _fuse_projection(self, x, weight, bn, project, relu, out_plain, out, scale2, shift2):
+        px, pconv, pbn = project
+        co, ci, kh, kw = weight.shape
+        pw = pconv.weight
+        if not (self.split and self.fuse_proj) or x.fmt != "f32s" or px.fmt != "f32s" or x.nchw or px.nchw:
+            return None
+        if (kh, kw) != (3, 3) or pbn is None or bn is None or pconv.bias is not None:
+            return None
+        if tuple(pw.shape[2:]) != (1, 1) or tuple(pconv.stride) != (2, 2) or tuple(pconv.padding) != (0, 0) or \
+                tuple(pconv.dilation) != (1, 1) or pconv.groups != 1:
+            return None
+        cp = int(pw.shape[1])
+        if int(pw.shape[0]) != co or cp != px.C or cp % 32 or px.c_off % 32 or px.B != x.B or ci % 32 or co % 32:
+            return None
+        if ((px.H - 1) // 2 + 1, (px.W - 1) // 2 + 1) != (x.H, x.W):
+            return None
+        out_pitch = (co + 31) // 32 * 32
+        if out is not None:
+            if out.nchw or out.C != co:
+                return None
+            out_pitch, out_plain = out.pitch, out.fmt != "f32s"
+        probe = ConvDesc(B=x.B, H=x.H, W=x.W, Cin=ci, Ho=x.H, Wo=x.W, Cout=co, KH=3, KW=3, stride=1, pad_h=1,
+                         pad_w=1, dil=1, in_layout=LAYOUT_NHWC, in_pitch=x.pitch, out_layout=LAYOUT_NHWC,
+                         out_pitch=out_pitch, OH=x.H, OW=x.W, oy_mul=1, ox_mul=1, relu=int(relu),
+                         dtype=DTYPE_F32S, flags=CONV_Y_PLAIN if out_plain else 0)
+        probe.proj.H, probe.proj.W, probe.proj.Cin, probe.proj.pitch = px.H, px.W, cp, px.pitch
+        if not self.lib.cn_conv2d_proj_supported(ctypes.byref(probe)):
+            return None
+        sources = [t for t in (weight, pw, bn.weight, bn.bias, bn.running_mean, bn.running_var,
+                               pbn.weight, pbn.bias, pbn.running_mean, pbn.running_var) if t is not None]
+        key = self._wkey("proj_f32s:%d:%d" % (x.exp, px.exp), sources)
+        hit = self.wcache.get(key)
+        if hit is None:
+            scp, shp = fold_bn(None, pbn, co, self.device)
+            got = fuse_projection_weights(weight.to(self.device), scale2, shift2, pw.to(self.device), scp, shp,
+                                          x.exp, px.exp)
+            if got is None:
+                self._wput(key, False)
+                return None
+            stored, shift, bump = got
+            n = self.lib.cn_packed_conv_weight_elems(co, cp, 1, 1, DTYPE_F32S)
+            wpk = torch.empty(n, device=self.device, dtype=torch.float32)
+            w4 = stored.reshape(co, cp, 1, 1).contiguous()
+            native.check(self.lib.cn_pack_conv_weight(native.ptr(w4), native.ptr(wpk), co, cp, 1, 1, DTYPE_F32S,
+                                                      native.stream_ptr()), "cn_pack_conv_weight")
+            w2p = None
+            if int(bump.max()) > 0:
+                w2s, factor = prescale_rows(weight.detach().to(device=self.device, dtype=torch.float32))
+                w2s = torch.ldexp(w2s, (-bump).view(-1, 1, 1, 1).expand_as(w2s)).contiguous()
+                factor = torch.ldexp(factor, bump)
+                n2 = self.lib.cn_packed_conv_weight_elems(co, ci, 3, 3, DTYPE_F32S)
+                w2k = torch.empty(n2, device=self.device, dtype=torch.float32)
+                native.check(self.lib.cn_pack_conv_weight(native.ptr(w2s), native.ptr(w2k), co, ci, 3, 3, DTYPE_F32S,
+                                                          native.stream_ptr()), "cn_pack_conv_weight")
+                w2p = (w2k, factor)
+            ev = torch.cuda.Event()
+            ev.record()
+            hit = (wpk, shift, ev, w2p)
+            self._wput(key, hit)
+        if hit is False:
+            return None
+        self.keep += [hit[0], hit[1], hit[3]]
+        self._pack_events.append(hit[2])
+        return dict(x=px, w=hit[0], shift=hit[1], cin=cp, w2=hit[3])
+
     @staticmethod
     def _narrow_form(kh, kw, padding, dilation, out_nchw, ci, co):
         return ci == 16 and co <= 32 and (kh, kw, padding, dilation) == (3, 3, 1, 1) and not out_nchw
@@ -301,14 +404,24 @@
 
     def conv(self, x, weight, bias=None, bn=None, relu=False, residual=None, stride=1,
              padding=0, dilation=1, out_nchw=False, out=None, wsources=None, out_plain=False,
-             pool=None, lid=None):
+             pool=None, lid=None, project=None):
         co, ci, kh, kw = weight.shape
         assert ci == x.C, (ci, x.C)
         lid = self._lid(lid)
+        use_s = self.split and not x.nchw and self._f32s_conv_form(kh, kw, stride, padding,
+                                                                  dilation, out_nchw, ci, co)
+        scale, shift = fold_bn(bias, bn, co, self.device)
+        proj = None
+        if project is not None:
+            assert residual is None and bias is None and not out_nchw and pool is None
+            if use_s and stride == 1 and padding == 1 and dilation == 1:
+                proj = self._fuse_projection(x, weight, bn, project, relu, out_plain, out, scale, shift)
+            if proj is None:
+                px, pconv, pbn = project
+                residual = self.conv(px, pconv.weight, bias=pconv.bias, bn=pbn, stride=pconv.stride[0],
+                                     padding=pconv.padding[0], dilation=pconv.dilation[0], lid=lid + "/proj")
         Ho = _out_size(x.H, kh, stride, padding, dilation)
         Wo = _out_size(x.W, kw, stride, padding, dilation)
-        use_s = self.split and not x.nchw and self._f32s_conv_form(kh, kw, stride, padding,
-                                                                  dilation, out_nchw, ci, co)
         if use_s and self._narrow_form(kh, kw, padding, dilation, out_nchw, ci, co) and residual is None:
             x, out_plain = self.plain(x), True
         fuse_pool = False
@@ -318,7 +431,8 @@
                              stride=stride, pad_h=padding, pad_w=padding, dil=dilation,
                              in_layout=LAYOUT_NCHW, out_layout=LAYOUT_NHWC, dtype=self.cdtype)
             fuse_pool = bool(self.lib.cn_stem_maxpool_supported(ctypes.byref(probe)))
-        scale, shift = fold_bn(bias, bn, co, self.device)
+        if proj is not None:
+            shift = proj["shift"]
         flags = 0
         stem_s = False
         if self.split and x.nchw and not use_s:
@@ -328,7 +442,10 @@
                              OH=Ho, OW=Wo, oy_mul=1, ox_mul=1,
                              flags=CONV_STEM_F32S | (CONV_STEM_MAXPOOL if fuse_pool else 0))
             stem_s = bool(self.lib.cn_stem_f32s_supported(ctypes.byref(probe)))
-        if use_s:
+        if use_s and proj is not None and proj["w2"] is not None:
+            wp, factor = proj["w2"]
+            cd = DTYPE_F32S
+        elif use_s:
             wp, factor = self._pack(weight, wsources, f32s=True)
             if x.fmt == "f32":
                 flags |= CONV_X_PLAIN
@@ -419,6 +536,14 @@
         fl = 2 * x.B * Ho * Wo * co * ci * kh * kw
         by = 4 * (x.B * x.H * x.W * ci + x.B * out.H * out.W * co * (2 if residual is not None else 1)
                   + co * ci * kh * kw)
+        if proj is not None:
+            assert use_s and out.fmt in ("f32s", "f32") and residual is None
+            px = proj["x"]
+            d.proj.x, d.proj.w = px.ptr().value, proj["w"].data_ptr()
+            d.proj.H, d.proj.W, d.proj.Cin, d.proj.pitch = px.H, px.W, proj["cin"], px.pitch
+            self.keep.append(px.t)
+            fl += 2 * x.B * Ho * Wo * co * proj["cin"]
+            by += 4 * (px.B * px.H * px.W * proj["cin"] + co * proj["cin"])
         self._emit_conv(d, x, wp, scale, shift, residual, out, dict(kind="conv", flops=fl, bytes=by))
         self.flops += fl
         if pool is not None and not fuse_pool:
@@ -1081,6 +1206,10 @@
     def drop_plans(self):
         self.__dict__["_plans"] = {}
 
+    def fuse_projections(self, enable=True):
+        self.__dict__["_fuse_proj"] = bool(enable)
+        return self
+
     def defer_heads(self, names=()):
         self.__dict__["_defer"] = tuple(names)
         return self
@@ -1154,7 +1283,8 @@
     def plan_for(self, B, H, W, device, deferred=None):
         cache = self.__dict__.setdefault("_plans", {})
         defer = () if deferred is False else self.deferred_names()
-        key = (B, H, W, str(device), self.compute_dtype, self.f32s, self.range_tracking_on, defer)
+        fuse_proj = self.__dict__.get("_fuse_proj", True)
+        key = (B, H, W, str(device), self.compute_dtype, self.f32s, self.range_tracking_on, fuse_proj, defer)
         plan = cache.pop(key, None)
         if plan is None:
             native.lib()
@@ -1162,7 +1292,8 @@
                 pb = PlanBuilder(device, B, H, W, dtype=self.compute_dtype,
                                  wcache=self.__dict__.setdefault("_wcache", {}), split=self.f32s,
                                  exps=self.__dict__.get("_exps"),
-                                 track=None if self.range_tracking_on else False, defer=defer)
+                                 track=None if self.range_tracking_on else False, defer=defer,
+                                 fuse_proj=fuse_proj)
                 x = pb.set_input(3)
                 outs = self.describe(pb, x)
             plan = Plan(pb, outs)
diff --git a/centernet_amd/native.py b/centernet_amd/native.py
--- a/centernet_amd/native.py
+++ b/centernet_amd/native.py
@@ -38,11 +38,16 @@
     _fields_ = [("x_mul", ctypes.c_float), ("res_mul", ctypes.c_float), ("range", ctypes.c_void_p)]
 
 
+class ConvProj(ctypes.Structure):
+    _fields_ = [("x", ctypes.c_void_p), ("w", ctypes.c_void_p), ("H", ctypes.c_int), ("W", ctypes.c_int),
+                ("Cin", ctypes.c_int), ("pitch", ctypes.c_int)]
+
+
 class ConvDesc(ctypes.Structure):
     _fields_ = [(n, ctypes.c_int) for n in (
         "B", "H", "W", "Cin", "Ho", "Wo", "Cout", "KH", "KW", "stride", "pad_h", "pad_w",
         "dil", "in_layout", "in_pitch", "out_layout", "out_pitch", "OH", "OW", "oy_mul",
-        "oy_add", "ox_mul", "ox_add", "relu", "dtype", "flags", "res_pitch")] + [("ctl", F32sCtl)]
+        "oy_add", "ox_mul", "ox_add", "relu", "dtype", "flags", "res_pitch")] + [("ctl", F32sCtl), ("proj", ConvProj)]
 
 
 class HeadOut(ctypes.Structure):
@@ -141,6 +146,8 @@
     lib.cn_pack_conv_weight.argtypes = [vp, vp, i, i, i, i, i, vp]
     lib.cn_conv2d_res_pitch_supported.restype = i
     lib.cn_conv2d_res_pitch_supported.argtypes = [ctypes.POINTER(ConvDesc)]
+    lib.cn_conv2d_proj_supported.restype = i
+    lib.cn_conv2d_proj_supported.argtypes = [ctypes.POINTER(ConvDesc)]
     lib.cn_conv2d_workspace_bytes.restype = sz
     lib.cn_conv2d_workspace_bytes.argtypes = [ctypes.POINTER(ConvDesc)]
     lib.cn_conv2d.restype = i
diff --git a/centernet_amd/networks/resnet.py b/centernet_amd/networks/resnet.py
--- a/centernet_amd/networks/resnet.py
+++ b/centernet_amd/networks/resnet.py
@@ -15,12 +15,11 @@
         self.conv2, self.bn2 = conv(planes, planes, 3), bn(planes)
 
     def describe(self, pb, x, out_plain=False):
-        res = x
+        out = pb.conv(x, self.conv1.weight, bn=self.bn1, relu=True, stride=self.stride, padding=1)
         if self.downsample is not None:
-            ds = self.downsample
-            res = pb.conv(x, ds[0].weight, bn=ds[1], stride=ds[0].stride[0])
-        out = pb.conv(x, self.conv1.weight, bn=self.bn1, relu=True, stride=self.stride, padding=1)
-        return pb.conv(out, self.conv2.weight, bn=self.bn2, relu=True, residual=res, padding=1,
+            return pb.conv(out, self.conv2.weight, bn=self.bn2, relu=True, padding=1, out_plain=out_plain,
+                           project=(x, self.downsample[0], self.downsample[1]))
+        return pb.conv(out, self.conv2.weight, bn=self.bn2, relu=True, residual=x, padding=1,
                        out_plain=out_plain)
 
 
diff --git a/include/centernet_amd.h b/include/centernet_amd.h
--- a/include/centernet_amd.h
+++ b/include/centernet_amd.h
@@ -91,6 +91,11 @@
                      unsigned long long *out, void *stream);
 int cn_calib_clock(unsigned long long *out, int ticks, void *stream);
 
+typedef struct cn_conv_proj {
+    const void *x;
+    const void *w;
+    int H, W, Cin, pitch;
+} cn_conv_proj;
 typedef struct cn_conv_desc {
     int B, H, W, Cin;
     int Ho, Wo, Cout;
@@ -104,7 +109,9 @@
     int flags;
     int res_pitch;
     cn_f32s_ctl ctl;
+    cn_conv_proj proj;
 } cn_conv_desc;
+int cn_conv2d_proj_supported(const cn_conv_desc *d);
 int cn_conv2d_res_pitch_supported(const cn_conv_desc *d);
 #define CN_CONV_X_PLAIN 1
 #define CN_CONV_Y_PLAIN 2
```

New measurement: 12390 img/s (median of 6 runs). Within noise of the previous version (+0.6%).
